# zsyOAOA/ResShift

Measured on AMD Instinct MI355X. Metric: images/sec (1x3x64x64 LR -> 3x256x256, 15-step ResShift sampling loop incl. VQ encode/decode), higher is better.
Workload: dtype f16x2 encoder + UNet (hi+lo fp16 pairs, 3 MFMAs per product: fp32-class) + f16 decoder (parity policy); 1 GPU; realsr_swinunet_realesrgan256: batch 32/GPU x 1 GPU, 1x3x64x64 LR -> 3x256x256, 15 steps, random-init weights; precision_policy=parity, parallelism=dp1 (batch sharded, one RCCL weight broadcast, no data-path collective)

## Files before the change

### include/resshift_hip.h

```cpp
#ifndef RESSHIFT_HIP_H
#define RESSHIFT_HIP_H
#include <stddef.h>
#include <stdint.h>

#ifdef __cplusplus
extern "C" {
#endif

#define RS_PREC_F16 0
#define RS_PREC_F32 1
#define RS_PREC_SPLIT 2
#define RS_MAX_LEVELS 8
#define RS_MAX_STEPS 64
#define RS_MAX_ROWS 64

typedef struct rs_engine rs_engine;

typedef struct rs_unet_config {
    int image_size, in_channels, model_channels, out_channels;
    int n_levels;
    int channel_mult[RS_MAX_LEVELS];
    int num_res_blocks[RS_MAX_LEVELS];
    int n_attn_res;
    int attention_resolutions[RS_MAX_LEVELS];
// ... 46 lines not shown
    float* x;
    float* pred_xstart;
    const float* y;
    const float* mask;
    const float* noise;
    const int* t;
    int B;
    int prec;
    void* stream;
} rs_step_args;

rs_engine* rs_create(const rs_config* cfg);
void rs_destroy(rs_engine* e);
const char* rs_last_error(void);

int rs_load_tensor(rs_engine* e, const char* state_dict_key, const float* host, const int64_t* shape, int ndim);
size_t rs_weight_bytes(rs_engine* e);
int rs_bind_weight_blob(rs_engine* e, void* dev, size_t bytes);
int rs_pack_weights(rs_engine* e);
int rs_bcast_weights(rs_engine* e, void* rccl_comm, int root, void* stream);
int rs_weights_ready(rs_engine* e);

int rs_unet_forward(rs_engine* e, const float* x, const int* t_host, const float* lq, const float* mask, float* out,
                    int B, int H, int W, int Hl, int Wl, int prec, void* stream);
int rs_vq_encode(rs_engine* e, const float* img, float* z, int B, int H, int W, int prec, void* stream);
int rs_vq_decode(rs_engine* e, const float* z, float* img, int32_t* idx_out, int B, int h, int w, int force_not_quantize,
                 int prec, void* stream);
int rs_bicubic(rs_engine* e, const float* y, float* out, int B, int C, int H, int W, int sf, void* stream);
int rs_sample(rs_engine* e, const rs_sample_args* a);
int rs_sample_begin(rs_engine* e, const rs_sample_args* a, float* x_T);
int rs_sample_step(rs_engine* e, const rs_step_args* s);
int rs_sample_end(rs_engine* e, const rs_sample_args* a, const float* x_0);
int rs_film_prewarm(rs_engine* e, const int* timesteps, int n, void* stream);
int rs_axpbypcz(const float* x, const float* z, const float* n, float* y, float a, float b, float c, long long count, void* stream);
int rs_axpbypcz_rows(const float* x, const float* z, const float* n, float* y, const float* a, const float* b, const float* c,
                     long long per_image_count, int B, void* stream);

typedef struct rs_noise_key {
    uint64_t seed;
    uint32_t stream;
    uint32_t reserved;
} rs_noise_key;
int rs_noise_fill(const rs_noise_key* keys, const int* draw, float* out, long long per_image_count, int B, void* stream);
int rs_sample_seeded(rs_engine* e, const rs_sample_args* a, const rs_noise_key* keys);
int rs_sample_begin_seeded(rs_engine* e, const rs_sample_args* a, float* x_T, const rs_noise_key* keys);
int rs_sample_step_seeded(rs_engine* e, const rs_step_args* s, const rs_noise_key* keys);

int rs_tile_accumulate(float* acc, float* count, const float* tile, int B, int C, int H, int W, int h0, int w0, int th, int tw,
                       void* stream);
int rs_tile_finalize(float* acc, const float* count, int B, int C, int H, int W, void* stream);
int rs_window_copy(const float* in, float* out, long long planes, int H, int W, int h0, int w0, int Ho, int Wo, float scale, void* stream);

typedef struct rs_tile_desc {
    const float* src;
    float* acc;
    float* count;
    int H, W, h0, w0, th, tw;
} rs_tile_desc;
int rs_tile_gather(const rs_tile_desc* desc, int n, int C_src, float* out_lq, float* out_mask, int Hp, int Wp, void* stream);
int rs_tile_scatter(const rs_tile_desc* desc, int n, int C, int sf, const float* tiles, int Hp_out, int Wp_out, void* stream);

int rs_tile_accumulate_weighted(float* acc, float* count, const float* tile, int B, int C, int H, int W, int h0, int w0, int th, int tw,
                                int Rh, int Rw, void* stream);
int rs_tile_scatter_weighted(const rs_tile_desc* desc, int n, int C, int sf, const float* tiles, int Hp_out, int Wp_out, int Rh, int Rw,
                             void* stream);

#define RS_COLOR_FIX_WAVELET 1
#define RS_COLOR_FIX_ADAIN 2
size_t rs_color_fix_work_bytes(int B, int C, int H, int W, int sf, int mode);
int rs_color_fix(const float* sr, const float* lq, float* out, int B, int C, int H, int W, int sf, int mode, void* work, size_t work_bytes,
                 void* stream);

int rs_u8_to_input(const void* src_u8_nhwc, float* dst_f32_nchw, int B, int H, int W, int C, void* stream);
int rs_output_to_u8(const float* sr_f32_nchw, const float* lq_f32_nchw, const float* mask_f32_n1hw, void* dst_u8_nhwc, int B, int H,
                    int W, int C, int bgr, void* stream);

size_t rs_arena_bytes(rs_engine* e);
long long rs_last_launch_count(rs_engine* e);
int rs_profile_enable(rs_engine* e, int on);
int rs_profile_get(rs_engine* e, double* out9);
int rs_profile_families(rs_engine* e, double* out, int cap);
int rs_profile_shapes(rs_engine* e, char* buf, int cap);
int rs_debug_enable(rs_engine* e, int on);
int rs_debug_count(rs_engine* e);
int rs_debug_info(rs_engine* e, int i, char* name, int name_cap, int* dims_bchw);
int rs_debug_fetch(rs_engine* e, int i, float* out_nchw_dev, void* stream);
int rs_debug_fetch_rows(rs_engine* e, int i, int b0, int nb, float* out_nchw_dev, void* stream);

int rs_op_conv2d(const void* x0, const void* x1, const float* w_ref_host, const float* bias_host, const void* res, void* y,
                 int B, int Hs, int Ws, int C0, int C1, int Cout, int KH, int KW, int stride, int pad_t, int pad_l, int Ho,
                 int Wo, int up, int act, int in_prec, int out_prec, int force_direct, void* stream);
int rs_op_conv2d_bench(const void* x0, const void* w_packed_dev, const float* bias_dev, const void* res, void* y, int B, int Hs,
                       int Ws, int Cin, int Cout, int KH, int KW, int stride, int pad, int Ho, int Wo, int up, int act, int in_prec,
                       int out_prec, int reps, float* ms_out, void* stream);
int rs_op_conv3x3_halo(const void* x, const float* coef_dev, int act_in, const float* w_ref_host, const float* bias_host, const void* res,
                       void* y, int B, int H, int W, int Cin, int Cout, int prec, float* ystats_dev, void* stream);
int rs_op_conv3x3_wino(const void* x, const float* coef_dev, int act_in, const float* w_ref_host, const float* bias_host, const void* res,
                       void* y, int B, int H, int W, int Cin, int Cout, float* ystats_dev, int reps, float* ms_out, void* stream);
int rs_op_conv3x3_halo_stats_px(int B, int H, int W, int Cin, int Cout, int prec);
int rs_op_gemm_nt(const void* a, const void* b, const float* bias_dev, void* y, int nz, int M, int N, int K, float scale,
                  int in_prec, int out_prec, void* stream);
int rs_op_groupnorm(const void* x, void* y, const float* gamma_host, const float* beta_host, const float* film_dev, int B, int HW,
                    int C, int groups, float eps, int act, int prec, void* stream);
int rs_op_window_attention(const void* qkv, void* out, const float* bias_table_host , int B, int H, int W,
                           int heads, int shift, int prec, void* stream);
int rs_op_window_attention_qkv(const void* x, const void* wqkv_dev, const float* bqkv_dev, const void* wproj_dev, const float* bproj_dev,
                               const void* res, void* out, const float* table_host, int B, int H, int W, int heads, int shift, void* stream);
int rs_op_window_attention_qkv_split(const void* x, const void* wqkv_dev, const float* bqkv_dev, const void* wproj_dev, const float* bproj_dev,
                                     const void* res, void* out, const float* table_host, const float* xcoef_dev, int B, int H, int W, int heads,
                                     int shift, void* stream);
int rs_op_ae_flash_attention(const void* q, const void* k, const void* vt, const float* bv_dev, void* o, int nz, int T, int C, void* stream);
int rs_op_ae_flash_attention_split(const void* q, const void* k, const void* vt, const float* bv_dev, void* o, int nz, int T, int C, void* stream);
int rs_op_swin_mlp(const void* x, const void* w1_dev, const float* b1_dev, const void* w2_dev, const float* b2_dev, const void* res, void* y,
                   int M, int E, int HD, void* stream);
int rs_op_swin_mlp_split(const void* x, const void* w1_dev, const float* b1_dev, const void* w2_dev, const float* b2_dev, const void* res, void* y,
                         int M, int E, int HD, void* stream);
int rs_op_swin_mlp_split_unembed(const void* x, const float* xcoef_dev, const void* w1_dev, const float* b1_dev, const void* w2cat_dev, const float* bcat_dev,
                                 void* y, int M, int HW, int E, int HD, int NO, void* stream);
int rs_op_softmax_rows(const float* s, void* out, long long nrows, int ncols, int out_prec, void* stream);
int rs_op_vq(const float* z, const float* codebook_dev, float* zq, int32_t* idx, long long N, int NE, int D, void* stream);
int rs_op_nchw_to_nhwc(const float* in, void* out, int B, int C, int HW, int out_prec, void* stream);
int rs_op_nhwc_to_nchw(const void* in, float* out, int B, int C, int HW, int in_prec, void* stream);
int rs_op_convert(const void* src, int src_prec, void* dst, int dst_prec, int C, long long npix, void* stream);

#ifdef __cplusplus
}
#endif
#endif
```

### resshift_amd/_lib.py

```python
from __future__ import annotations

import ctypes as C
import os

import torch

HERE = os.path.dirname(os.path.abspath(__file__))
LIB_PATH = os.environ.get("RESSHIFT_HIP_LIB") or os.path.join(HERE, "libresshift_hip.so")

RS_PREC_F16 = 0
RS_PREC_F32 = 1
RS_PREC_SPLIT = 2
RS_MAX_LEVELS = 8
RS_MAX_STEPS = 64
RS_MAX_ROWS = 64
RS_COLOR_FIX_WAVELET = 1
RS_COLOR_FIX_ADAIN = 2
COLOR_FIX_MODES = {"wavelet": RS_COLOR_FIX_WAVELET, "adain": RS_COLOR_FIX_ADAIN}


class UNetConfig(C.Structure):
    _fields_ = [
        ("image_size", C.c_int), ("in_channels", C.c_int), ("model_channels", C.c_int), ("out_channels", C.c_int),
        ("n_levels", C.c_int),
# ... 31 lines not shown
        ("B", C.c_int), ("h", C.c_int), ("w", C.c_int), ("sf", C.c_int), ("steps", C.c_int),
        ("inv_std", C.c_float * RS_MAX_STEPS), ("coef1", C.c_float * RS_MAX_STEPS), ("coef2", C.c_float * RS_MAX_STEPS),
        ("sigma", C.c_float * RS_MAX_STEPS), ("tmap", C.c_int * RS_MAX_STEPS),
        ("prior_scale", C.c_float), ("scale_factor", C.c_float),
        ("prec_encode", C.c_int), ("prec_decode", C.c_int), ("prec_unet", C.c_int * RS_MAX_STEPS),
        ("stream", C.c_void_p),
    ]


class StepArgs(C.Structure):
    _fields_ = [
        ("sched", C.POINTER(SampleArgs)), ("x", C.c_void_p), ("pred_xstart", C.c_void_p), ("y", C.c_void_p), ("mask", C.c_void_p),
        ("noise", C.c_void_p), ("t", C.POINTER(C.c_int)), ("B", C.c_int), ("prec", C.c_int), ("stream", C.c_void_p),
    ]


class TileDesc(C.Structure):
    _fields_ = [("src", C.c_void_p), ("acc", C.c_void_p), ("count", C.c_void_p),
                ("H", C.c_int), ("W", C.c_int), ("h0", C.c_int), ("w0", C.c_int), ("th", C.c_int), ("tw", C.c_int)]


class NoiseKey(C.Structure):
    _fields_ = [("seed", C.c_uint64), ("stream", C.c_uint32), ("reserved", C.c_uint32)]


def noise_keys(keys):
    arr = (NoiseKey * max(1, len(keys)))()
    for d, k in zip(arr, keys):
        if isinstance(k, NoiseKey):
            d.seed, d.stream, d.reserved = k.seed, k.stream, k.reserved
            continue
        seed, stream = (k if isinstance(k, (tuple, list)) else (k, 0))
        if not 0 <= int(stream) < 2 ** 32:
            raise ValueError(f"noise key stream {stream} does not fit 32 bits")
        d.seed, d.stream, d.reserved = int(seed) % 2 ** 64, int(stream), 0
    return arr


_P, _I, _F, _LL, _SZ = C.c_void_p, C.c_int, C.c_float, C.c_longlong, C.c_size_t

SIGNATURES = {
    "rs_create": (_P, [C.POINTER(Config)]),
    "rs_destroy": (None, [_P]),
    "rs_last_error": (C.c_char_p, []),
    "rs_load_tensor": (_I, [_P, C.c_char_p, _P, C.POINTER(C.c_int64), _I]),
    "rs_weight_bytes": (_SZ, [_P]),
    "rs_bind_weight_blob": (_I, [_P, _P, _SZ]),
    "rs_pack_weights": (_I, [_P]),
    "rs_bcast_weights": (_I, [_P, _P, _I, _P]),
    "rs_weights_ready": (_I, [_P]),
    "rs_unet_forward": (_I, [_P, _P, C.POINTER(C.c_int), _P, _P, _P, _I, _I, _I, _I, _I, _I, _P]),
    "rs_vq_encode": (_I, [_P, _P, _P, _I, _I, _I, _I, _P]),
    "rs_vq_decode": (_I, [_P, _P, _P, _P, _I, _I, _I, _I, _I, _P]),
    "rs_bicubic": (_I, [_P, _P, _P, _I, _I, _I, _I, _I, _P]),
    "rs_sample": (_I, [_P, C.POINTER(SampleArgs)]),
    "rs_sample_begin": (_I, [_P, C.POINTER(SampleArgs), _P]),
    "rs_sample_step": (_I, [_P, C.POINTER(StepArgs)]),
    "rs_sample_end": (_I, [_P, C.POINTER(SampleArgs), _P]),
    "rs_film_prewarm": (_I, [_P, C.POINTER(C.c_int), _I, _P]),
    "rs_axpbypcz": (_I, [_P, _P, _P, _P, _F, _F, _F, _LL, _P]),
    "rs_axpbypcz_rows": (_I, [_P, _P, _P, _P, C.POINTER(C.c_float), C.POINTER(C.c_float), C.POINTER(C.c_float), _LL, _I, _P]),
    "rs_noise_fill": (_I, [C.POINTER(NoiseKey), C.POINTER(C.c_int), _P, _LL, _I, _P]),
    "rs_sample_seeded": (_I, [_P, C.POINTER(SampleArgs), C.POINTER(NoiseKey)]),
    "rs_sample_begin_seeded": (_I, [_P, C.POINTER(SampleArgs), _P, C.POINTER(NoiseKey)]),
    "rs_sample_step_seeded": (_I, [_P, C.POINTER(StepArgs), C.POINTER(NoiseKey)]),
    "rs_tile_accumulate": (_I, [_P, _P, _P] + [_I] * 8 + [_P]),
    "rs_tile_finalize": (_I, [_P, _P, _I, _I, _I, _I, _P]),
    "rs_window_copy": (_I, [_P, _P, _LL, _I, _I, _I, _I, _I, _I, _F, _P]),
    "rs_tile_gather": (_I, [C.POINTER(TileDesc), _I, _I, _P, _P, _I, _I, _P]),
    "rs_tile_scatter": (_I, [C.POINTER(TileDesc), _I, _I, _I, _P, _I, _I, _P]),
    "rs_tile_accumulate_weighted": (_I, [_P, _P, _P] + [_I] * 10 + [_P]),
    "rs_tile_scatter_weighted": (_I, [C.POINTER(TileDesc), _I, _I, _I, _P, _I, _I, _I, _I, _P]),
    "rs_color_fix_work_bytes": (_SZ, [_I] * 6),
    "rs_color_fix": (_I, [_P, _P, _P] + [_I] * 6 + [_P, _SZ, _P]),
    "rs_u8_to_input": (_I, [_P, _P, _I, _I, _I, _I, _P]),
    "rs_output_to_u8": (_I, [_P, _P, _P, _P, _I, _I, _I, _I, _I, _P]),
    "rs_arena_bytes": (_SZ, [_P]),
    "rs_last_launch_count": (_LL, [_P]),
    "rs_profile_enable": (_I, [_P, _I]),
    "rs_profile_get": (_I, [_P, C.POINTER(C.c_double)]),
    "rs_profile_families": (_I, [_P, C.POINTER(C.c_double), _I]),
    "rs_profile_shapes": (_I, [_P, C.c_char_p, _I]),
    "rs_debug_enable": (_I, [_P, _I]),
    "rs_debug_count": (_I, [_P]),
    "rs_debug_info": (_I, [_P, _I, C.c_char_p, _I, C.POINTER(C.c_int)]),
    "rs_debug_fetch": (_I, [_P, _I, _P, _P]),
    "rs_debug_fetch_rows": (_I, [_P, _I, _I, _I, _P, _P]),
    "rs_op_conv2d": (_I, [_P, _P, _P, _P, _P, _P] + [_I] * 18 + [_P]),
    "rs_op_conv2d_bench": (_I, [_P, _P, _P, _P, _P] + [_I] * 16 + [C.POINTER(C.c_float), _P]),
    "rs_op_conv3x3_halo_stats_px": (_I, [_I, _I, _I, _I, _I, _I]),
    "rs_op_conv3x3_halo": (_I, [_P, _P, _I, _P, _P, _P, _P, _I, _I, _I, _I, _I, _I, _P, _P]),
    "rs_op_conv3x3_wino": (_I, [_P, _P, _I, _P, _P, _P, _P, _I, _I, _I, _I, _I, _P, _I, C.POINTER(C.c_float), _P]),
    "rs_op_gemm_nt": (_I, [_P, _P, _P, _P, _I, _I, _I, _I, _F, _I, _I, _P]),
    "rs_op_groupnorm": (_I, [_P, _P, _P, _P, _P, _I, _I, _I, _I, _F, _I, _I, _P]),
    "rs_op_window_attention": (_I, [_P, _P, _P, _I, _I, _I, _I, _I, _I, _P]),
    "rs_op_window_attention_qkv": (_I, [_P, _P, _P, _P, _P, _P, _P, _P, _I, _I, _I, _I, _I, _P]),
    "rs_op_window_attention_qkv_split": (_I, [_P, _P, _P, _P, _P, _P, _P, _P, _P, _I, _I, _I, _I, _I, _P]),
    "rs_op_swin_mlp": (_I, [_P, _P, _P, _P, _P, _P, _P, _I, _I, _I, _P]),
    "rs_op_ae_flash_attention": (_I, [_P, _P, _P, _P, _P, _I, _I, _I, _P]),
    "rs_op_ae_flash_attention_split": (_I, [_P, _P, _P, _P, _P, _I, _I, _I, _P]),
    "rs_op_swin_mlp_split": (_I, [_P, _P, _P, _P, _P, _P, _P, _I, _I, _I, _P]),
    "rs_op_swin_mlp_split_unembed": (_I, [_P, _P, _P, _P, _P, _P, _P, _I, _I, _I, _I, _I, _P]),
    "rs_op_softmax_rows": (_I, [_P, _P, _LL, _I, _I, _P]),
    "rs_op_vq": (_I, [_P, _P, _P, _P, _LL, _I, _I, _P]),
    "rs_op_nchw_to_nhwc": (_I, [_P, _P, _I, _I, _I, _I, _P]),
    "rs_op_nhwc_to_nchw": (_I, [_P, _P, _I, _I, _I, _I, _P]),
    "rs_op_convert": (_I, [_P, _I, _P, _I, _I, _LL, _P]),
}

_lib = None


def load() -> C.CDLL:
    global _lib
    if _lib is not None:
        return _lib
    if not os.path.exists(LIB_PATH):
        raise RuntimeError(
            f"{LIB_PATH} is missing: build it with `python -m resshift_amd.build` (hipcc, gfx950). "
            "There is no CPU fallback for the ResShift hot path."
        )
    try:
        lib = C.CDLL(LIB_PATH, mode=C.RTLD_GLOBAL)
    except OSError as e:
        raise RuntimeError(f"cannot load {LIB_PATH}: {e}") from e
    for name, (res, args) in SIGNATURES.items():
        fn = getattr(lib, name)
        fn.restype = res
        fn.argtypes = args
    _lib = lib
    return lib


def last_error() -> str:
    return load().rs_last_error().decode()


def check(rc: int, what: str = "") -> None:
    if rc != 0:
        raise RuntimeError(f"resshift_hip {what} failed (rc={rc}): {last_error()}")


def current_stream_ptr() -> int:
    if torch.cuda.is_available():
        return int(torch.cuda.current_stream().cuda_stream)
    return 0


def window_copy(x, h0=0, w0=0, ho=None, wo=None, scale=1.0, out=None):
    import torch

    if not x.is_cuda:
        raise RuntimeError("window_copy needs a device tensor: the host mirror does not fall back to CPU arithmetic")
    x = x.to(torch.float32).contiguous()
    H, W = x.shape[-2:]
    ho = H if ho is None else ho
    wo = W if wo is None else wo
    planes = x.numel() // (H * W)
    want = (*x.shape[:-2], ho, wo)
    if out is None:
        out = torch.empty(*want, device=x.device, dtype=torch.float32)
    elif out.dtype != torch.float32 or tuple(out.shape) != want or not out.is_contiguous() or out.device != x.device:
        raise ValueError(f"window_copy: `out` must be a contiguous float32 tensor of shape {want} on {x.device} "
                         f"(got {out.dtype}, {tuple(out.shape)}, contiguous={out.is_contiguous()}, {out.device})")
    check(load().rs_window_copy(x.data_ptr(), out.data_ptr(), planes, H, W, h0, w0, ho, wo, float(scale), current_stream_ptr()), "rs_window_copy")
    return out


def _tile_descs(rows):
    arr = (TileDesc * len(rows))()
    for d, r in zip(arr, rows):
        d.src, d.acc, d.count, d.H, d.W, d.h0, d.w0, d.th, d.tw = r
    return arr


# ... 66 lines not shown
```

### resshift_amd/build.py

```python
from __future__ import annotations

import concurrent.futures as cf
import hashlib
import os
import subprocess
import sys

HERE = os.path.dirname(os.path.abspath(__file__))
CSRC = os.path.join(HERE, "csrc")
OBJ = os.path.join(CSRC, "build" + ("_" + hashlib.sha256(os.environ["RS_BUILD_DEFS"].encode()).hexdigest()[:8] if os.environ.get("RS_BUILD_DEFS") else ""))
LIB = os.environ.get("RS_BUILD_OUT") or os.path.join(HERE, "libresshift_hip.so")
SOURCES = ["igemm.hip", "igemm2.hip", "igemm3.hip", "igemm4.hip", "igemm4s.hip", "wino.hip", "igemm_split.hip", "swin_mlp.hip", "direct_conv.hip", "norm_attn.hip", "win_attn_split.hip", "ae_attn.hip", "ae_attn_split.hip", "elementwise.hip", "colorfix.hip", "engine.hip"]
HEADERS = ["common.h", "igemm_common.h", "igemm4_kernel.h", "gn_tail.h", "philox.h", os.path.join("..", "..", "include", "resshift_hip.h")]
HIPCC = os.environ.get("HIPCC", "/opt/rocm/bin/hipcc")
FLAGS = ["--offload-arch=gfx950", "-O3", "-std=c++17", "-fPIC", "-Wno-unused-result"]
FLAGS += [f"-D{d}" for d in os.environ.get("RS_BUILD_DEFS", "").split() if d]
if os.environ.get("RS_BUILD_ABLATE"):
    FLAGS.append("-DRS_SPLIT_ABLATE")


def _digest() -> str:
    h = hashlib.sha256()
    for f in SOURCES + HEADERS:
        with open(os.path.join(CSRC, f), "rb") as fh:
            h.update(fh.read())
    h.update(" ".join(FLAGS).encode())
    return h.hexdigest()


def _compile(src: str) -> str:
    obj = os.path.join(OBJ, src.replace(".hip", ".o"))
    cmd = [HIPCC, *FLAGS, "-c", os.path.join(CSRC, src), "-o", obj]
    r = subprocess.run(cmd, capture_output=True, text=True)
    if r.returncode != 0:
        raise RuntimeError(f"hipcc failed for {src}:\n{r.stderr[-4000:]}")
    return obj


def build(force: bool = False, verbose: bool = True) -> str:
    os.makedirs(OBJ, exist_ok=True)
    stamp = LIB + ".stamp"
    dig = _digest()
    if not force and os.path.exists(LIB) and os.path.exists(stamp) and open(stamp).read().strip() == dig:
        return LIB
    if verbose:
        print(f"[resshift_amd.build] compiling {len(SOURCES)} HIP sources for gfx950 ...", flush=True)
    with cf.ThreadPoolExecutor(max_workers=min(8, len(SOURCES))) as ex:
        objs = list(ex.map(_compile, SOURCES))
    cmd = [HIPCC, "--offload-arch=gfx950", "-shared", "-fPIC", "-o", LIB, *objs]
    r = subprocess.run(cmd, capture_output=True, text=True)
    if r.returncode != 0:
        raise RuntimeError(f"link failed:\n{r.stderr[-4000:]}")
    chk = subprocess.run([sys.executable, "-c", f"import ctypes; ctypes.CDLL({LIB!r})"], capture_output=True, text=True)
    if chk.returncode != 0:
        raise RuntimeError(f"built library does not load:\n{chk.stderr[-2000:]}")
    with open(stamp, "w") as fh:
        fh.write(dig)
    if verbose:
        print(f"[resshift_amd.build] built {LIB}", flush=True)
    return LIB


def build_testhooks(verbose: bool = False) -> str:
    build(force=False, verbose=verbose)
    out = os.path.join(HERE, "libresshift_hip_testhooks.so")
    stamp = out + ".stamp"
    dig = _digest() + "+hooks"
    if os.path.exists(out) and os.path.exists(stamp) and open(stamp).read().strip() == dig:
        return out
    objs = [os.path.join(OBJ, s.replace(".hip", ".o")) for s in SOURCES if s != "engine.hip"]
    if not all(os.path.exists(o) for o in objs):
        os.makedirs(OBJ, exist_ok=True)
        with cf.ThreadPoolExecutor(max_workers=min(8, len(SOURCES))) as ex:
            list(ex.map(_compile, [s for s in SOURCES if s != "engine.hip"]))
    hobj = os.path.join(OBJ, "engine_testhooks.o")
    r = subprocess.run([HIPCC, *FLAGS, "-DRS_TEST_HOOKS", "-c", os.path.join(CSRC, "engine.hip"), "-o", hobj], capture_output=True, text=True)
    if r.returncode != 0:
        raise RuntimeError(f"hipcc failed for engine.hip (-DRS_TEST_HOOKS):\n{r.stderr[-4000:]}")
    r = subprocess.run([HIPCC, "--offload-arch=gfx950", "-shared", "-fPIC", "-o", out, *objs, hobj], capture_output=True, text=True)
    if r.returncode != 0:
        raise RuntimeError(f"link failed:\n{r.stderr[-4000:]}")
    with open(stamp, "w") as fh:
        fh.write(dig)
    return out


if __name__ == "__main__":
    build(force="--force" in sys.argv)
```

### resshift_amd/csrc/common.h

```cpp
#pragma once
#include <hip/hip_runtime.h>
#include <stdint.h>
#include <type_traits>

typedef _Float16 f16;
typedef f16 f16x4 __attribute__((ext_vector_type(4)));
typedef f16 f16x8 __attribute__((ext_vector_type(8)));
typedef float f32x4 __attribute__((ext_vector_type(4)));

enum RsDType { RS_F16 = 0, RS_F32 = 1, RS_F16S = 2 };
enum RsAct { RS_ACT_NONE = 0, RS_ACT_GELU = 1, RS_ACT_SILU = 2 };

static inline size_t rs_dtype_size(int dt) { return dt == RS_F16 ? 2 : 4; }
static inline size_t rs_dtype_chan_bytes(int dt) { return dt == RS_F32 ? 4 : 2; }

struct h2s { unsigned short bits; };
#define RS_LO_SCALE 2048.0f
#define RS_LO_INV 4.8828125e-4f
__host__ __device__ inline void rs_split(float x, f16& hi, f16& lo) {
    hi = (f16)x;
    lo = (f16)((x - (float)hi) * RS_LO_SCALE);
}
__device__ __forceinline__ float rs_join(f16 hi, f16 lo) { return fmaf((float)lo, RS_LO_INV, (float)hi); }
template <typename T> struct Store { static constexpr int PM = 1; static constexpr bool FAST = false; };
// ... 82 lines not shown
    const rs_f32x2 es = {copysignf(e.x, x.x), copysignf(e.y, x.y)};
    return __builtin_elementwise_fma(es, hx, hx);
}
__device__ __forceinline__ void rs_split2(rs_f32x2 v, rs_f16x2& h, rs_f16x2& l) {
    h = __builtin_convertvector(v, rs_f16x2);
    l = __builtin_convertvector((v - __builtin_convertvector(h, rs_f32x2)) * RS_LO_SCALE, rs_f16x2);
}
template <int ACT, bool FAST> __device__ __forceinline__ float rs_act_t(float x) {
    if constexpr (ACT == RS_ACT_GELU) return FAST ? rs_gelu_fast(x) : rs_gelu(x);
    else if constexpr (ACT == RS_ACT_SILU) return FAST ? rs_silu_fast(x) : rs_silu(x);
    else return x;
}

template <typename T> struct Vec8;
template <> struct Vec8<f16> {
    f16x8 v;
    __device__ __forceinline__ void load(const f16* p, int lo = 0) { v = *(const f16x8*)p; }
    __device__ __forceinline__ void store(f16* p, int lo = 0) const { *(f16x8*)p = v; }
    __device__ __forceinline__ float get(int i) const { return (float)v[i]; }
    __device__ __forceinline__ void set(int i, float x) { v[i] = (f16)x; }
};
template <> struct Vec8<float> {
    f32x4 a, b;
    __device__ __forceinline__ void load(const float* p, int lo = 0) { a = *(const f32x4*)p; b = *(const f32x4*)(p + 4); }
    __device__ __forceinline__ void store(float* p, int lo = 0) const { *(f32x4*)p = a; *(f32x4*)(p + 4) = b; }
    __device__ __forceinline__ float get(int i) const { return i < 4 ? a[i] : b[i - 4]; }
    __device__ __forceinline__ void set(int i, float x) { if (i < 4) a[i] = x; else b[i - 4] = x; }
};
template <> struct Vec8<h2s> {
    f16x8 h, l;
    __device__ __forceinline__ void load(const h2s* p, int lo) { h = *(const f16x8*)p; l = *(const f16x8*)((const f16*)p + lo); }
    __device__ __forceinline__ void store(h2s* p, int lo) const { *(f16x8*)p = h; *(f16x8*)((f16*)p + lo) = l; }
    __device__ __forceinline__ float get(int i) const { return rs_join(h[i], l[i]); }
    __device__ __forceinline__ void set(int i, float x) { f16 a, b; rs_split(x, a, b); h[i] = a; l[i] = b; }
};


struct GNTail {
    const float* gamma; const float* beta;
    const float* film;
    int film_ld;
    float* coef;
    unsigned* ticket;
    int expected;
    int C, groups, HW;
    float eps;
    const float* st0; int S0, ld0, n0;
    const float* st1; int S1, ld1;
    const float* stg; int Sg;
};


struct IGemmParams {
    const void* x0;
    const void* x1;
    const void* w;
    const float* bias;
    const void* res;
    void* y;
    int C0, C1, ld0, ld1;
    int B, Hs, Ws, up;
    int Ho, Wo, KH, KW, stride, pad_t, pad_l;
    int Cout, ldy, ldres;
    int M, Ktot;
    int act;
    float out_scale;
    long long bs_x0, bs_w, bs_y, bs_res;
    int splitk;
    float* partial;
    unsigned x_bytes, w_bytes;
    int sh_howo, sh_wo;
    int dbg;
    int no_halo;
    const float* xcoef;
    int xact;
    float* ystats;
    int ystats_ld;
    GNTail tail;
    const void* sx; const void* sw; const float* sbias;
    int sC, sld;
    unsigned sx_bytes, sw_bytes;
    int osc, ooy, oox;
    const void* ww;
};

#if defined(__HIPCC__)
__device__ __forceinline__ long long rs_out_m(const IGemmParams& p, long long m) {
    if (p.osc != 2) return m;
    const int hw = p.Ho * p.Wo;
    const int b = (int)(m / hw), r = (int)(m - (long long)b * hw);
    const int oy = r / p.Wo, ox = r - oy * p.Wo;
    return ((long long)b * (2 * p.Ho) + 2 * oy + p.ooy) * (2 * p.Wo) + 2 * ox + p.oox;
}
#endif

struct DirectConvParams {
    const void* x0; const void* x1;
    const float* w;
    const float* bias;
    void* y;
    int C0, C1, ld0, ld1;
    int B, Hs, Ws, up, Ho, Wo, KH, KW, stride, pad_t, pad_l;
    int Cout, ldy, act;
};

struct GNParams {
    const void* x; void* y;
    const float* gamma; const float* beta;
    const float* film;
    int film_ld;
    float* partial;
    int B, HW, C, ldx, ldy, S, groups;
    float eps; int act;
    float* coef;
    const float* cpartial;
    int cp_ld;
    const float* cpartial2;
    int cp2_ld, cp2_S, cp_n0;
    unsigned* ticket;
};

struct WinAttnParams {
    const void* qkv;
    void* out;
    const float* bias_t;
    const float* bias_n;
    const float* bias_c;
    int B, H, W, heads, shift, ldq, ldo;
    float scale;
    const void* x;
    const void* wqkv;
    const float* bqkv;
    int ldx;
    const void* wproj;
    const float* bproj;
    const void* res;
    int ldres;
    const float* xcoef;
    float* ystats;
    int ystats_ld;
    GNTail tail;
};
```

### resshift_amd/csrc/engine.hip

```cpp
#include "common.h"
#include "../../include/resshift_hip.h"
#include <dlfcn.h>
#include <algorithm>
#include <array>
#include <cmath>
#include <cstdio>
#include <cstring>
#include <functional>
#include <map>
#include <string>
#include <unordered_map>
#include <vector>

extern "C" {
int rs_igemm_launch(const IGemmParams* p, int in_dt, int out_dt, int nz, hipStream_t st);
int rs_igemm_splitk_plan(int M, int Cout, int Ktot, int in_dt);
int rs_igemm4_pick(const IGemmParams* p, int in_dt, int out_dt, int nz, int* TW, int* BC);
int rs_igemm4_plan(const IGemmParams* p, int in_dt, int out_dt, int nz, int* TW, int* BC, int* SEG, int* SK);
int rs_igemm4_stats_px(const IGemmParams* p, int in_dt);
int rs_wino_plan(const IGemmParams* p, int in_dt, int out_dt, int nz);
int rs_wino_launch(const IGemmParams* p, hipStream_t st);
size_t rs_wino_weight_bytes(int Cin, int Cout);
float rs_wino_pack(const float* w_ref, int Cin, int Cout, void* dst);
int rs_wino_stats_px();
int rs_wino_tiles(const IGemmParams* p);
int rs_igemm_split_stats_px(const IGemmParams* p, int splitk);
int rs_direct_conv_launch(const DirectConvParams* p, int in_dt, int out_dt, hipStream_t st);
int rs_head_conv_launch(const void* x, int in_dt, const float* coef_dev, const float* w_dev, const float* bias_dev, float* y, int B, int H, int W, int C,
                        int ldx, int Cout, int ldy, hipStream_t st);
int rs_groupnorm_launch(const GNParams* p, int dt, int apply_slabs, hipStream_t st);
int rs_win_attn_launch(const WinAttnParams* p, int dt, hipStream_t st);
int rs_softmax_rows_launch(const float* s, void* out, int out_dt, long long nrows, int ncols, long long lds_, long long ldo, hipStream_t st);
int rs_nchw_to_nhwc_launch(const float* in, void* out, int out_dt, int B, int C, int HW, int ldo, int coff, float scale, hipStream_t st);
int rs_nhwc_to_nchw_launch(const void* in, int in_dt, float* out, int B, int C, int HW, int ldi, int coff, hipStream_t st);
int rs_axpbypcz_launch(const float* x, const float* z, const float* n, float* y, float a, float b, float c, long long cnt, hipStream_t st);
int rs_axpbypcz_rows_launch(const float* x, const float* z, const float* n, float* y, const float* a, const float* b, const float* c, long long per,
                            int B, hipStream_t st);
int rs_axpbypcz_seeded_launch(const float* x, const float* z, float* y, const float* a, const float* b, const float* c, const rs_noise_key* keys,
                              const rs_noise_key* keys_dev, const int* draw, long long per, int B, hipStream_t st);
int rs_film_gather_launch(const float* const* rows, int B, int total, float* out, hipStream_t st);
int rs_nchw_to_nhwc_rows_launch(const float* in, void* out, int out_dt, int B, int C, int HW, int ldo, int coff, const float* scale, hipStream_t st);
int rs_clamp_launch(float* x, float lo, float hi, long long cnt, hipStream_t st);
int rs_win_attn_qkv_supported(int heads, int E);
int rs_win_attn_qkv_launch(const WinAttnParams* p, hipStream_t st);
int rs_win_attn_qkv_split_launch(const WinAttnParams* p, hipStream_t st);
int rs_ae_flash_supported(int C, int T);
int rs_ae_flash_launch(const void* q, int ldq, const void* k, int ldk, const void* vt, const float* bv, void* o, int ldo, int nz, int T, int C,
                       float scale, hipStream_t st);
int rs_ae_flash_split_supported(int C, int T);
int rs_ae_flash_split_launch(const void* q, int ldq, const void* k, int ldk, const void* vt, const float* bv, void* o, int ldo, int nz, int T, int C,
                             float scale, hipStream_t st);
int rs_swin_mlp_supported(int E, int HD);
int rs_swin_mlp_split_launch(const void* x, const void* w1, const float* b1, const void* w2, const float* b2, const void* res, void* y, int M, int ldx,
                             int ldres, int ldy, int E, int HD, const float* xcoef, int HW, float* ystats, int ystats_ld, const GNTail* tail, hipStream_t st);
int rs_swin_mlp_split_launch_n(const void* x, const void* w1, const float* b1, const void* w2, const float* b2, const void* res, void* y, int M, int ldx,
                               int ldres, int ldy, int E, int HD, int NO, const float* xcoef, int HW, float* ystats, int ystats_ld, const GNTail* tail,
                               hipStream_t st);
int rs_swin_mlp_split_unembed_supported(int E, int HD, int NO);
int rs_swin_mlp_launch(const void* x, const void* w1, const float* b1, const void* w2, const float* b2, const void* res, void* y, int M, int ldx,
                       int ldres, int ldy, int E, int HD, const float* xcoef, int HW, float* ystats, int ystats_ld, hipStream_t st);
int rs_small_linear_launch(const float* x, const float* w, const float* bias, float* y, int R, int K, int N, int silu_in, int silu_out, hipStream_t st);
int rs_bicubic_launch(const float* in, void* out, int out_dt, int B, int C, int H, int W, int sf, int ldo, hipStream_t st);
int rs_vq_launch(const float* z, const float* codebook, float* zq, int* idx, long long N, int NE, int D, hipStream_t st);
int rs_copy_channels_launch(const void* src, int lds_, void* dst, int ldd, int C, long long npix, int dt, hipStream_t st);
int rs_convert_launch(const void* src, int src_dt, void* dst, int dst_dt, int C, long long npix, hipStream_t st);
}

namespace {

thread_local std::string g_err;
int fail(const std::string& m) { g_err = m; return -1; }

struct HostTensor { std::vector<float> data; std::vector<int64_t> shape; };

template <class FH, class FL>
static void frag_major_fill(int N, int K, f16* dst, bool with_lo, FH hi, FL lo) {
    const int KS = K / 32, parts = with_lo ? 2 : 1;
    for (int nb = 0; nb < N / 16; ++nb)
        for (int ks = 0; ks < KS; ++ks)
            for (int lane = 0; lane < 64; ++lane)
                for (int e = 0; e < 8; ++e) {
                    const int n = 16 * nb + (lane & 15), k = 32 * ks + 8 * (lane >> 4) + e;
                    const size_t o = (((size_t)(nb * KS + ks) * parts) * 64 + lane) * 8 + e;
                    dst[o] = hi(n, k);
                    if (with_lo) dst[o + 512] = lo(n, k);
                }
}
static void rs_pack_frag_major(const float* w, int N, int K, f16* out16, f16* outsplit) {
    if (out16) frag_major_fill(N, K, out16, false, [&](int n, int k) { return (f16)w[(size_t)n * K + k]; }, [&](int, int) { return (f16)0.f; });
    if (outsplit)
        frag_major_fill(N, K, outsplit, true, [&](int n, int k) { f16 h, l; rs_split(w[(size_t)n * K + k], h, l); return h; },
                        [&](int n, int k) { f16 h, l; rs_split(w[(size_t)n * K + k], h, l); return l; });
}
static void* frag_major_from_device_rows(const void* wdev, int N, int K, int ld, int lo_off) {
    std::vector<f16> rows((size_t)N * ld), out((size_t)N * K * (lo_off >= 0 ? 2 : 1));
    if (hipMemcpy(rows.data(), wdev, rows.size() * sizeof(f16), hipMemcpyDeviceToHost) != hipSuccess) return nullptr;
    frag_major_fill(N, K, out.data(), lo_off >= 0, [&](int n, int k) { return rows[(size_t)n * ld + k]; },
                    [&](int n, int k) { return rows[(size_t)n * ld + (lo_off >= 0 ? lo_off : 0) + k]; });
    void* d = nullptr;
    if (hipMalloc(&d, out.size() * sizeof(f16)) != hipSuccess) return nullptr;
    (void)hipMemcpy(d, out.data(), out.size() * sizeof(f16), hipMemcpyHostToDevice);
    return d;
}

struct View {
    void* p = nullptr; int B = 0, H = 0, W = 0, C = 0, ld = 0, dt = RS_F16;
    float* st = nullptr; int stS = 0, stld = 0;
    int st_prod = -1;
    float* st2 = nullptr; int st2S = 0, st2ld = 0, st_n0 = 0;
// ... 215 lines not shown
            (void)hipEventRecord(e0, st);
        }
        if (sp) check(rs_win_attn_qkv_split_launch(&p, st), "win_attn_qkv_split");
        else check(rs_win_attn_qkv_launch(&p, st), "win_attn_qkv");
        if (e1) (void)hipEventRecord(e1, st);
    }
    void ae_flash(const void* q, int ldq, const void* k, int ldk, const void* vt, const float* bv, void* o, int ldo, int nz, int T, int C, float scale,
                  int dt = RS_F16) {
        const int sp = dt == RS_F16S;
        const double fl = 4.0 * (double)nz * (double)T * (double)T * (double)C;
        igemm_flops[sp ? 2 : 0] += fl;
        fam_note(sp ? F_AEFLASH_S : F_AEFLASH, fl, T, T, C, nz);
        igemm_bytes += (sp ? 4.0 : 2.0) * 4.0 * (double)nz * T * C;
        ++igemm_launches;
        hipEvent_t e0, e1;
        bracket(prof, st, e0, e1);
        if (sp) check(rs_ae_flash_split_launch(q, ldq, k, ldk, vt, bv, o, ldo, nz, T, C, scale, st), "ae_flash_attn_split");
        else check(rs_ae_flash_launch(q, ldq, k, ldk, vt, bv, o, ldo, nz, T, C, scale, st), "ae_flash_attn");
        if (e1) (void)hipEventRecord(e1, st);
    }
    void swin_mlp(const void* x, const void* w1, const float* b1, const void* w2, const float* b2, const void* res, void* y, int M, int ldx,
                  int ldres, int ldy, int E, int HD, const float* xcoef = nullptr, int HW = 0, int dt = RS_F16, float* ystats = nullptr,
                  int ystats_ld = 0, const GNTail* tail = nullptr, int NO = 0) {
        const int sp = dt == RS_F16S;
        if (NO <= 0) NO = E;
        const double fl = 2.0 * (double)M * ((double)E * HD + (double)NO * (NO != E ? HD + E : HD));
        igemm_flops[sp ? 2 : 0] += fl;
        fam_note(sp ? F_SWINMLP_S : F_SWINMLP, fl, M, NO, HD);
        igemm_bytes += (sp ? 4.0 : 2.0) * ((double)M * (E * ((res || NO != E) ? 2.0 : 1.0) + NO) + (double)E * HD + (double)NO * (NO != E ? HD + E : HD));
        ++igemm_launches;
        hipEvent_t e0 = nullptr, e1 = nullptr;
        if (prof && prof->on) {
            if (prof->used + 2 > prof->ev.size()) {
                const size_t old = prof->ev.size();
                prof->ev.resize(old + 1024);
                for (size_t i = old; i < prof->ev.size(); ++i) (void)hipEventCreate(&prof->ev[i]);
            }
            e0 = prof->ev[prof->used++]; e1 = prof->ev[prof->used++];
            (void)hipEventRecord(e0, st);
        }
        if (sp) check(rs_swin_mlp_split_launch_n(x, w1, b1, w2, b2, res, y, M, ldx, ldres, ldy, E, HD, NO, xcoef, HW, ystats, ystats_ld, tail, st), "swin_mlp_split");
        else check(rs_swin_mlp_launch(x, w1, b1, w2, b2, res, y, M, ldx, ldres, ldy, E, HD, xcoef, HW, ystats, ystats_ld, st), "swin_mlp");
        if (e1) (void)hipEventRecord(e1, st);
    }
};

}

#ifdef RS_TEST_HOOKS
static bool rs_fake_device() {
    static const bool fake = []() {
        if (!getenv("RS_FAKE_DEVICE")) return false;
        int n = 0;
        const hipError_t e = hipGetDeviceCount(&n);
        return e == hipErrorNoDevice || (e == hipSuccess && n == 0);
    }();
    return fake;
}
#else
static constexpr bool rs_fake_device() { return false; }
#endif

struct rs_engine {
    rs_config cfg;
    std::unordered_map<std::string, HostTensor> host;
    Blob blob;
    size_t blob_bytes = 0;
    bool bound = false, ready = false;
    std::string build_err;
    std::string split_err;
    bool split_ok = true;
    std::vector<unsigned char> big_w;
    int conv_count = 0;
    unsigned char* big_w_dev = nullptr;
    bool big(const ConvW& c) const { return c.idx >= 0 && c.idx < (int)big_w.size() && big_w[c.idx] != 0; }
    Arena arena;
    long long last_launches = 0;
    Exec::Prof prof, prof_gn;
    double last_flops[3] = {0.0, 0.0, 0.0}, last_igemm_ms = 0.0, last_igemm_bytes = 0.0, last_gn_ms = 0.0, last_gn_bytes = 0.0;
    double last_fam[Exec::F_COUNT][3] = {};
    std::string last_shapes;
    long long last_igemm_launches = 0, last_gn_launches = 0;
    bool debug = false;
    std::vector<TraceRec> trace;
    rs_noise_key* keys_dev = nullptr; size_t keys_cap = 0;
    const rs_noise_key* stage_keys(const rs_noise_key* keys, int B, hipStream_t st) {
        if (rs_fake_device()) return (const rs_noise_key*)(uintptr_t)4096;
        if ((size_t)B > keys_cap) {
            (void)hipStreamSynchronize(st);
            if (keys_dev) (void)hipFree(keys_dev);
            keys_dev = nullptr; keys_cap = 0;
            if (hipMalloc((void**)&keys_dev, (size_t)B * sizeof(rs_noise_key)) != hipSuccess) return nullptr;
            keys_cap = (size_t)B;
        }
        if (hipMemcpyWithStream(keys_dev, keys, (size_t)B * sizeof(rs_noise_key), hipMemcpyHostToDevice, st) != hipSuccess) return nullptr;
        return keys_dev;
    }
    char* cap_base = nullptr; size_t cap_bytes = 0; bool cap_host = false;
    void free_capture() {
        if (cap_base) { if (cap_host) free(cap_base); else (void)hipFree(cap_base); }
        cap_base = nullptr; cap_bytes = 0; trace.clear();
    }
    std::vector<TailPlan> tail_plan;
    std::vector<UBlock> in_blocks, out_blocks;
    ResBlockW mid_res1, mid_res2; BasicLayerW mid_swin;
    std::vector<ConvW> fe_convs, fe_downs;
    GNW out_norm; ConvW out_conv;
    ConvW te0, te2;
    std::vector<int> skip_ch, h_ch;
    int film_total = 0, fe_out_ch = 0;
    std::vector<ResBlockW*> film_blocks;
    std::map<int, float*> film_cache;
    ConvW enc_in, enc_out, dec_in, dec_out, quant_conv, post_quant_conv;
    std::vector<AELevel> enc_levels, dec_levels;
    ResBlockW enc_mid1, enc_mid2, dec_mid1, dec_mid2;
    AttnW enc_attn, dec_attn;
    GNW enc_norm, dec_norm;
    float* codebook = nullptr;

    std::map<std::string, std::function<bool(HostTensor&)>> derived;
    const HostTensor* find(const std::string& k) {
        auto it = host.find(k);
        if (it == host.end()) {
            auto d = derived.find(k);
            if (d != derived.end()) {
                HostTensor t;
                if (d->second(t)) it = host.emplace(k, std::move(t)).first;
            }
        }
        if (it == host.end()) { if (build_err.empty()) build_err = "missing state_dict key: " + k; return nullptr; }
        return &it->second;
    }
    float* add_f32(const std::string& key, size_t n) {
        return (float*)blob.add(n * sizeof(float), [&](char* dst) {
            const HostTensor* t = find(key);
            if (!t) return;
            if (t->data.size() != n) { if (build_err.empty()) build_err = "bad size for " + key; return; }
            memcpy(dst, t->data.data(), n * sizeof(float));
        });
    }
    ConvW add_conv(const std::string& prefix, int Cin, int Cout, int KH, int KW, bool has_bias = true, bool force_direct = false, bool head = false) {
        ConvW c; c.Cin = Cin; c.Cout = Cout; c.KH = KH; c.KW = KW;
        c.idx = conv_count++;
        if ((int)big_w.size() < conv_count) big_w.resize(conv_count, 0);
        const int cidx = c.idx;
        c.direct = force_direct;
        c.CinP = c.direct ? Cin : (Cin + 7) / 8 * 8;
        const int CinP = c.CinP;
        const size_t K = (size_t)KH * KW * CinP, n = (size_t)KH * KW * Cin * Cout, np = K * Cout;
        const std::string wkey = prefix + ".weight";
        auto get = [&]() -> const float* {
            const HostTensor* t = find(wkey);
            if (!t) return nullptr;
            if (t->data.size() != n) { if (build_err.empty()) build_err = "bad size for " + wkey; return nullptr; }
            return t->data.data();
        };
        if (c.direct) {
            c.wd = (float*)blob.add(n * 4, [&](char* dst) {
                const float* w = get(); if (!w) return;
                float* o = (float*)dst;
                for (int co = 0; co < Cout; ++co)
                    for (int ci = 0; ci < Cin; ++ci)
                        for (int t = 0; t < KH * KW; ++t)
                            o[((size_t)t * Cin + ci) * Cout + co] = w[((size_t)co * Cin + ci) * KH * KW + t];
            });
        } else {
// ... 345 lines not shown
    ResBlockW add_resnet(const std::string& p, int Cin, int Cout) {
        ResBlockW r; r.Cin = Cin; r.Cout = Cout;
        r.n1 = add_gn(p + ".norm1", Cin);
        r.c1 = add_conv(p + ".conv1", Cin, Cout, 3, 3);
        r.n2 = add_gn(p + ".norm2", Cout);
        r.c2 = add_conv(p + ".conv2", Cout, Cout, 3, 3);
        r.has_skip = Cin != Cout;
        if (r.has_skip) r.skip = add_conv(p + ".nin_shortcut", Cin, Cout, 1, 1);
        return r;
    }
    AttnW add_attn(const std::string& p, int C) {
        AttnW a; a.C = C;
        a.norm = add_gn(p + ".norm", C);
        a.q = add_conv(p + ".q", C, C, 1, 1);
        a.k = add_conv(p + ".k", C, C, 1, 1);
        a.v = add_conv(p + ".v", C, C, 1, 1);
        a.proj = add_conv(p + ".proj_out", C, C, 1, 1);
        return a;
    }
    void build_ae() {
        const rs_ae_config& a = cfg.ae;
        enc_levels.clear(); dec_levels.clear();
        enc_in = add_conv("encoder.conv_in", a.in_channels, a.ch, 3, 3);
        int block_in = a.ch;
        for (int l = 0; l < a.n_levels; ++l) {
            AELevel L;
            block_in = a.ch * (l == 0 ? 1 : a.ch_mult[l - 1]);
            const int block_out = a.ch * a.ch_mult[l];
            for (int i = 0; i < a.num_res_blocks[l]; ++i) {
                L.blocks.push_back(add_resnet("encoder.down." + std::to_string(l) + ".block." + std::to_string(i), block_in, block_out));
                block_in = block_out;
            }
            if (l != a.n_levels - 1) {
                L.has_resample = true;
                L.resample = add_conv("encoder.down." + std::to_string(l) + ".downsample.conv", block_in, block_in, 3, 3);
            }
            enc_levels.push_back(L);
        }
        enc_mid1 = add_resnet("encoder.mid.block_1", block_in, block_in);
        enc_attn = add_attn("encoder.mid.attn_1", block_in);
        enc_mid2 = add_resnet("encoder.mid.block_2", block_in, block_in);
        enc_norm = add_gn("encoder.norm_out", block_in);
        enc_out = add_conv("encoder.conv_out", block_in, a.z_channels, 3, 3, true, false, true);
        quant_conv = add_conv("quant_conv", a.z_channels, a.embed_dim, 1, 1, true, true);
        post_quant_conv = add_conv("post_quant_conv", a.embed_dim, a.z_channels, 1, 1, true, true);
        block_in = a.ch * a.ch_mult[a.n_levels - 1];
        dec_in = add_conv("decoder.conv_in", a.z_channels, block_in, 3, 3);
        dec_mid1 = add_resnet("decoder.mid.block_1", block_in, block_in);
        dec_attn = add_attn("decoder.mid.attn_1", block_in);
        dec_mid2 = add_resnet("decoder.mid.block_2", block_in, block_in);
        dec_levels.resize(a.n_levels);
        for (int l = a.n_levels - 1; l >= 0; --l) {
            AELevel L;
            const int block_out = a.ch * a.ch_mult[l];
            for (int i = 0; i <= a.num_res_blocks[l]; ++i) {
                L.blocks.push_back(add_resnet("decoder.up." + std::to_string(l) + ".block." + std::to_string(i), block_in, block_out));
                block_in = block_out;
            }
            if (l != 0) {
                L.has_resample = true;
                L.resample = add_conv("decoder.up." + std::to_string(l) + ".upsample.conv", block_in, block_in, 3, 3);
                L.has_upf = add_upfold("decoder.up." + std::to_string(l) + ".upsample.conv", block_in, L.upf);
            }
            dec_levels[l] = L;
        }
        dec_norm = add_gn("decoder.norm_out", block_in);
        dec_out = add_conv("decoder.conv_out", block_in, a.out_ch, 3, 3, true, false, true);
        codebook = add_f32("quantize.embedding.weight", (size_t)a.n_embed * a.embed_dim);
    }
    size_t build(char* base, bool fill) {
        blob.base = base; blob.off = 0; blob.fill = fill;
        build_err.clear();
        split_err.clear();
        if (fill) blob.staging.assign(blob_bytes, 0);
        (void)blob.add(256, [](char*) {});
        conv_count = 0;
        if (fill) std::fill(big_w.begin(), big_w.end(), 0);
        if (cfg.has_unet) build_unet();
        if (cfg.has_ae) build_ae();
        big_w_dev = (unsigned char*)blob.add((size_t)conv_count, [&](char* dst) { memcpy(dst, big_w.data(), (size_t)conv_count); });
        return (blob.off + 255) & ~(size_t)255;
    }

    static IGemmParams conv_params(const ConvW& w, const View& x, const View* x1, const View& y, int stride, int pad_t, int pad_l, int up,
                                   int act, const View* res, float out_scale) {
        const int C1 = x1 ? x1->C : 0;
        IGemmParams p{};
        p.x0 = x.p; p.x1 = x1 ? x1->p : nullptr; p.w = w.w_for(x.dt); p.bias = w.bias;
        p.res = res ? res->p : nullptr; p.y = y.p;
        p.C0 = x.C; p.C1 = C1; p.ld0 = x.ld; p.ld1 = x1 ? x1->ld : 0;
        p.B = x.B; p.Hs = x.H; p.Ws = x.W; p.up = up; p.Ho = y.H; p.Wo = y.W; p.KH = w.KH; p.KW = w.KW;
        p.stride = stride; p.pad_t = pad_t; p.pad_l = pad_l; p.Cout = w.Cout; p.ldy = y.ld; p.ldres = res ? res->ld : 0;
        p.M = y.B * y.H * y.W; p.Ktot = w.KH * w.KW * (x.C + C1); p.act = act; p.out_scale = out_scale;
        p.splitk = 1;
        p.ww = (x.dt == RS_F16S && !x1) ? w.ww : nullptr;
        return p;
    }
    bool halo_conv(const ConvW& w, const View& x, const View& y, const View* res, int* sk = nullptr, int* seg = nullptr, bool folded = false,
                   bool* wino = nullptr) const {
        if (wino) *wino = false;
        if (w.direct || (x.dt != RS_F16 && x.dt != RS_F16S) || y.dt != x.dt || x.C != w.CinP) return false;
        if (x.dt == RS_F16S && big(w)) return false;
        const IGemmParams p = conv_params(w, x, nullptr, y, 1, 1, 1, 1, 0, res, 1.f);
        if (!folded && rs_wino_plan(&p, x.dt, y.dt, 1)) {
            if (sk) *sk = 1;
            if (seg) *seg = 0;
            if (wino) *wino = true;
            return true;
        }
        int tw, bc, sg = 0, k = 1;
        if (!rs_igemm4_plan(&p, x.dt, y.dt, 1, &tw, &bc, &sg, &k)) return false;
        if (sk) *sk = k;
        if (seg) *seg = sg;
        return true;
    }
    void conv(Exec& ex, const ConvW& w, const View& x, const View* x1, const View& y, int stride, int pad_t, int pad_l, int up,
              int act, const View* res, float out_scale = 1.f, const float* xcoef = nullptr, int xact = RS_ACT_NONE,
              const ConvW* skw = nullptr, const View* skx = nullptr) {
        const int C1 = x1 ? x1->C : 0;
        int splitk = 1;
        float* partial = nullptr;
        if (!w.direct) {
            const int M = y.B * y.H * y.W;
            int sk4 = 1;
            if (!x1 && w.KH == 3 && stride == 1 && pad_t == 1 && pad_l == 1 && up == 1 && halo_conv(w, x, y, res, &sk4, nullptr, skw != nullptr)) splitk = sk4;
            else splitk = rs_igemm_splitk_plan(M, w.Cout, w.KH * w.KW * (x.C + C1), x.dt);
            if (splitk > 1) partial = (float*)ex.raw((size_t)splitk * M * w.Cout * sizeof(float));
        }
        View xcat;
        if (!w.direct && x1 && x.dt == RS_F16S) {
            xcat = ex.T(x.B, x.H, x.W, x.C + C1, x.dt);
            if (!ex.dry) {
                ex.check(rs_copy_channels_launch(x.p, x.ld, xcat.p, xcat.ld, x.C, x.pixels(), x.dt, ex.st), "concat copy");
                ex.check(rs_copy_channels_launch(x1->p, x1->ld, xcat.slice(x.C, C1).p, xcat.ld, C1, x.pixels(), x.dt, ex.st), "concat copy");
            }
            conv(ex, w, xcat, nullptr, y, stride, pad_t, pad_l, up, act, res, out_scale);
            return;
        }
        if (ex.dry) return;
        if (x.C + C1 != w.CinP) { if (!ex.err) { ex.err = -3; g_err = "conv input channels do not match the packed weights"; } return; }
        if (w.direct) {
            DirectConvParams p{};
            p.x0 = x.p; p.x1 = x1 ? x1->p : nullptr; p.w = w.wd; p.bias = w.bias; p.y = y.p;
            p.C0 = x.C; p.C1 = C1; p.ld0 = x.ld; p.ld1 = x1 ? x1->ld : 0;
            p.B = x.B; p.Hs = x.H; p.Ws = x.W; p.up = up; p.Ho = y.H; p.Wo = y.W; p.KH = w.KH; p.KW = w.KW;
            p.stride = stride; p.pad_t = pad_t; p.pad_l = pad_l; p.Cout = w.Cout; p.ldy = y.ld; p.act = act;
            if (res) { ex.err = -3; g_err = "direct conv has no residual path"; return; }
            ex.check(rs_direct_conv_launch(&p, x.dt, y.dt, ex.st), "direct_conv");
        } else {
            IGemmParams p = conv_params(w, x, x1, y, stride, pad_t, pad_l, up, act, res, out_scale);
            p.no_halo = (x.dt == RS_F16S && big(w)) ? 1 : 0;
            p.splitk = splitk; p.partial = partial;
            p.xcoef = xcoef; p.xact = xact;
            if (skw) { p.sx = skx->p; p.sw = skw->w_for(x.dt); p.sbias = skw->bias; p.sC = skx->C; p.sld = skx->ld; p.ww = nullptr; }
            if (y.st) {
                const bool halo = !x1 && w.KH == 3 && stride == 1 && pad_t == 1 && pad_l == 1 && up == 1 && halo_conv(w, x, y, res, nullptr, nullptr, skw != nullptr);
                if (halo || (!x1 && x.dt == RS_F16S && y.dt == RS_F16S)) { p.ystats = y.st; p.ystats_ld = y.stld; }
                else { ex.err = -3; g_err = "output statistics requested from a conv whose kernel cannot produce them"; return; }
                (void)ex.fill_tail(y.st_prod, y.B, p.tail);
            }
            if (!p.w) { ex.err = -3; g_err = "weights for this precision were not packed (enable_f16/enable_f32/enable_split)"; return; }
            ex.igemm(p, x.dt, y.dt, 1, "igemm");
        }
    }
    void zero(Exec& ex, const View& v) {
        if (ex.dry) return;
        const hipError_t e = hipMemsetAsync(v.p, 0, (size_t)v.B * v.H * v.W * v.ld * rs_dtype_size(v.dt), ex.st);
        ex.check(e == hipSuccess ? 0 : -1, "memset");
    }
    void conv3(Exec& ex, const ConvW& w, const View& x, const View& y, const View* res = nullptr, int act = 0, const float* xcoef = nullptr,
               int xact = RS_ACT_NONE, const ConvW* skw = nullptr, const View* skx = nullptr) {
        conv(ex, w, x, nullptr, y, 1, 1, 1, 1, act, res, 1.f, xcoef, xact, skw, skx);
    }
    bool skip_fold(const Exec& ex, const ResBlockW& r, const View& X, const View& h1, const View& Y) const {
        static const bool on = []() { const char* e = getenv("RS_SKIP_FOLD"); return !(e && e[0] == '0'); }();
        static const bool fold = []() { const char* e = getenv("RS_GN_CONV_FOLD"); return !(e && e[0] == '0'); }();
        static const bool on16 = []() { const char* e = getenv("RS_SKIP_FOLD_F16"); return !(e && e[0] == '0'); }();
        if (!on || !fold || !r.has_skip || (X.dt != RS_F16S && !(X.dt == RS_F16 && on16)) || Y.dt != X.dt) return false;
// ... 908 lines not shown

int rs_bcast_weights(rs_engine* e, void* rccl_comm, int root, void* stream) {
    if (!e || !e->bound || !rccl_comm) return fail("rs_bcast_weights: bind a weight blob first and pass an RCCL communicator");
    typedef int (*bcast_t)(const void*, void*, size_t, int, int, void*, hipStream_t);
    static bcast_t fn = []() -> bcast_t {
        void* h = dlopen("librccl.so", RTLD_NOW | RTLD_GLOBAL);
        if (!h) h = dlopen("librccl.so.1", RTLD_NOW | RTLD_GLOBAL);
        return h ? (bcast_t)dlsym(h, "ncclBroadcast") : nullptr;
    }();
    if (!fn) return fail("rs_bcast_weights: librccl.so (ncclBroadcast) not found");
    const int rc = fn(e->blob.base, e->blob.base, e->blob_bytes,  1, root, rccl_comm, (hipStream_t)stream);
    if (rc != 0) return fail("rs_bcast_weights: ncclBroadcast failed (ncclResult_t " + std::to_string(rc) + ")");
    e->ready = false;
    return 0;
}

int rs_pack_weights(rs_engine* e) {
    if (!e || !e->bound) return fail("rs_pack_weights: bind a weight blob first");
    char* base = e->blob.base;
    e->build(base, true);
    e->collect_film_blocks();
    if (!e->build_err.empty()) { e->blob.staging.clear(); e->blob.staging.shrink_to_fit(); return fail(e->build_err); }
    e->split_ok = e->split_err.empty();
    {
        const uint32_t flags = e->split_ok ? 1u : 0u;
        memcpy(e->blob.staging.data(), &flags, sizeof flags);
    }
    if (hipMemcpy(base, e->blob.staging.data(), e->blob_bytes, hipMemcpyHostToDevice) != hipSuccess) return fail("hipMemcpy of weight blob failed");
    e->blob.staging.clear(); e->blob.staging.shrink_to_fit();
    e->blob.fill = false;
    e->host.clear();
    for (auto& kv : e->film_cache) (void)hipFree(kv.second);
    e->film_cache.clear();
    e->ready = true;
    return 0;
}

int rs_weights_ready(rs_engine* e) {
    if (!e || !e->bound) return fail("rs_weights_ready: bind a weight blob first");
    uint32_t flags = 0;
    if (rs_fake_device()) { e->split_ok = true; e->ready = true; return 0; }
    if (hipMemcpy(&flags, e->blob.base, sizeof flags, hipMemcpyDeviceToHost) != hipSuccess) return fail("rs_weights_ready: cannot read the blob header");
    e->split_ok = (flags & 1u) != 0;
    if (e->conv_count > 0 && e->big_w_dev &&
        hipMemcpy(e->big_w.data(), e->big_w_dev, (size_t)e->conv_count, hipMemcpyDeviceToHost) != hipSuccess) return fail("rs_weights_ready: cannot read the per-layer flags");
    for (auto& kv : e->film_cache) (void)hipFree(kv.second);
    e->film_cache.clear();
    e->ready = true;
    return 0;
}

size_t rs_arena_bytes(rs_engine* e) { return e ? e->arena.cap : 0; }

int rs_profile_enable(rs_engine* e, int on) { if (!e) return -1; e->prof.on = on != 0; return 0; }
int rs_profile_get(rs_engine* e, double* out) {
    if (!e || !out) return -1;
    out[0] = e->last_flops[0]; out[1] = e->last_flops[1]; out[2] = e->last_igemm_ms; out[3] = (double)e->last_igemm_launches;
    out[4] = e->last_igemm_bytes; out[5] = e->last_flops[2];
    out[6] = e->last_gn_ms; out[7] = (double)e->last_gn_launches; out[8] = e->last_gn_bytes;
    return 0;
}

int rs_profile_families(rs_engine* e, double* out, int cap) {
    if (!e || !out || cap < 3 * Exec::F_COUNT) return -1;
    for (int f = 0; f < Exec::F_COUNT; ++f) { out[3 * f] = e->last_fam[f][0]; out[3 * f + 1] = e->last_fam[f][1]; out[3 * f + 2] = e->last_fam[f][2]; }
    return Exec::F_COUNT;
}

int rs_profile_shapes(rs_engine* e, char* buf, int cap) {
    if (!e) return -1;
    const int need = (int)e->last_shapes.size() + 1;
    if (buf && cap > 0) { const int n = std::min(cap - 1, need - 1); memcpy(buf, e->last_shapes.data(), n); buf[n] = 0; }
    return need;
}

int rs_debug_enable(rs_engine* e, int on) {
    if (!e) return -1;
    e->debug = on != 0;
    if (!e->debug) {
        if (e->cap_base && !e->cap_host) (void)hipDeviceSynchronize();
        e->free_capture();
    }
    e->trace.clear();
    return 0;
}
int rs_debug_count(rs_engine* e) { return e ? (int)e->trace.size() : 0; }
int rs_debug_info(rs_engine* e, int i, char* name, int cap, int* dims ) {
    if (!e || i < 0 || i >= (int)e->trace.size()) return -1;
    const TraceRec& t = e->trace[i];
    snprintf(name, cap, "%s", t.name.c_str());
    dims[0] = t.B; dims[1] = t.C; dims[2] = t.H; dims[3] = t.W;
    return 0;
}
int rs_debug_fetch(rs_engine* e, int i, float* out_nchw, void* stream) {
    if (!e || i < 0 || i >= (int)e->trace.size() || !e->cap_base) return -1;
    const TraceRec& t = e->trace[i];
    const size_t bytes = (size_t)t.B * t.C * t.H * t.W * sizeof(float);
    return hipMemcpyAsync(out_nchw, e->cap_base + t.off, bytes, hipMemcpyDefault, (hipStream_t)stream) == hipSuccess ? 0 : -1;
}
int rs_debug_fetch_rows(rs_engine* e, int i, int b0, int nb, float* out_nchw, void* stream) {
    if (!e || i < 0 || i >= (int)e->trace.size() || !e->cap_base) return -1;
    const TraceRec& t = e->trace[i];
    if (b0 < 0 || nb < 1 || b0 > t.B - nb) return -2;
    const size_t per = (size_t)t.C * t.H * t.W * sizeof(float);
    return hipMemcpyAsync(out_nchw, e->cap_base + t.off + (size_t)b0 * per, (size_t)nb * per, hipMemcpyDefault, (hipStream_t)stream) == hipSuccess ? 0 : -1;
}
long long rs_last_launch_count(rs_engine* e) { return e ? e->last_launches : 0; }

int rs_unet_forward(rs_engine* e, const float* x, const int* t_host, const float* lq, const float* mask, float* out, int B, int H, int W,
                    int Hl, int Wl, int prec, void* stream) {
    if (!e || !e->cfg.has_unet) return fail("engine has no UNet");
    {
        const int sh = e->cfg.unet.n_levels - 1;
        if ((H % (8 << sh)) || (W % (8 << sh))) return fail("UNet input H/W must be multiples of 8*2^(levels-1)");
    }
    hipStream_t st = (hipStream_t)stream;
    if (!e->ready) return fail("weights are not ready");
    if (B < 1 || !x || !out || !t_host) return fail("rs_unet_forward: bad batch / null tensor");
    if (e->cfg.unet.cond_lq && !lq) return fail("rs_unet_forward: this UNet is conditioned on lq (cond_lq) but lq is NULL");
    if (e->cfg.unet.cond_mask && !mask) return fail("rs_unet_forward: this UNet is conditioned on a mask (cond_mask) but mask is NULL");
    if (e->cfg.unet.cond_lq && e->fe_convs.empty() && (Hl != H || Wl != W))
        return fail("rs_unet_forward: without a feature extractor lq must have the latent resolution");
    if (!e->fe_convs.empty() && ((Hl >> (int)e->fe_convs.size()) != H || (Wl >> (int)e->fe_convs.size()) != W))
        return fail("rs_unet_forward: lq resolution does not match the feature extractor's down-sampling");
    bool mixed = false;
    for (int b = 1; b < B; ++b) mixed |= t_host[b] != t_host[0];
    if (mixed && B > RS_MAX_ROWS) return fail("rs_unet_forward: unequal timesteps in a batch of more than RS_MAX_ROWS (" + std::to_string(RS_MAX_ROWS) + ") images");
    std::vector<const float*> rows(mixed ? B : 1);
    for (size_t b = 0; b < rows.size(); ++b)
        if (!(rows[b] = e->film_row(t_host[b], st))) return fail("FiLM table allocation failed");
    return e->run(st, [&](Exec& ex) {
        View feat; const View* fp = nullptr;
        if (!e->fe_convs.empty()) { feat = e->feature_extract(ex, lq, mask, B, Hl, Wl, prec); fp = &feat; }
        if (!mixed) e->unet_body(ex, x, 1.0f, fp, lq, mask, Hl, Wl, out, B, H, W, prec, rows[0]);
        else e->unet_body(ex, x, 1.0f, fp, lq, mask, Hl, Wl, out, B, H, W, prec, e->film_table(ex, rows.data(), B), e->film_total);
    });
}

int rs_vq_encode(rs_engine* e, const float* img, float* z, int B, int H, int W, int prec, void* stream) {
    if (!e || !e->cfg.has_ae) return fail("engine has no autoencoder");
    hipStream_t st = (hipStream_t)stream;
    return e->run(st, [&](Exec& ex) {
        View in = ex.T(B, H, W, e->enc_in.CinP, prec);
        e->zero(ex, in);
        if (!ex.dry) ex.check(rs_nchw_to_nhwc_launch(img, in.p, prec, B, e->cfg.ae.in_channels, H * W, in.ld, 0, 1.f, st), "img->nhwc");
        e->encode_body(ex, in, z, prec);
    });
}

int rs_vq_decode(rs_engine* e, const float* z, float* img, int32_t* idx_out, int B, int h, int w, int force_not_quantize, int prec,
                 void* stream) {
    if (!e || !e->cfg.has_ae) return fail("engine has no autoencoder");
    hipStream_t st = (hipStream_t)stream;
    return e->run(st, [&](Exec& ex) { e->decode_body(ex, z, 1.0f, img, idx_out, B, h, w, force_not_quantize, prec); });
}

int rs_bicubic(rs_engine* e, const float* y, float* out, int B, int C, int H, int W, int sf, void* stream) {
    if (!e) return fail("null engine");
    hipStream_t st = (hipStream_t)stream;
    const bool was_ready = e->ready;
    e->ready = true;
    const int rc = e->run(st, [&](Exec& ex) {
        View t = ex.T(B, H * sf, W * sf, C, RS_F32);
        if (ex.dry) return;
        ex.check(rs_bicubic_launch(y, t.p, RS_F32, B, C, H, W, sf, t.ld, st), "bicubic");
        ex.check(rs_nhwc_to_nchw_launch(t.p, RS_F32, out, B, C, H * sf * W * sf, t.ld, 0, st), "bicubic->nchw");
// ... 307 lines not shown
            }
    void* wdev = dev_copy(o.data(), o.size() * 2);
    float* bias = bias_host ? (float*)dev_copy(bias_host, Cout * 4) : nullptr;
    IGemmParams p{};
    p.x0 = x; p.w = wdev; p.bias = bias; p.res = res; p.y = y; p.C0 = Cin; p.ld0 = Cin; p.B = B; p.Hs = H; p.Ws = W; p.up = 1; p.Ho = H; p.Wo = W;
    p.KH = 3; p.KW = 3; p.stride = 1; p.pad_t = 1; p.pad_l = 1; p.Cout = Cout; p.ldy = Cout; p.ldres = Cout; p.M = B * H * W; p.Ktot = (int)K;
    p.out_scale = 1.f; p.splitk = 1; p.xcoef = coef_dev; p.xact = act_in;
    int tw, bc, seg, sk, rc;
    float* part = nullptr;
    if (!rs_igemm4_plan(&p, prec, prec, 1, &tw, &bc, &seg, &sk)) rc = fail("shape is not eligible for the halo kernel");
    else {
        p.splitk = sk;
        if (sk > 1) { (void)hipMalloc((void**)&part, (size_t)sk * p.M * Cout * sizeof(float)); p.partial = part; }
        p.ystats = ystats_dev; p.ystats_ld = Cout;
        rc = rs_igemm_launch(&p, prec, prec, 1, st);
    }
    (void)hipStreamSynchronize(st);
    if (part) (void)hipFree(part);
    if (wdev) (void)hipFree(wdev);
    if (bias) (void)hipFree(bias);
    return rc;
}

int rs_op_conv3x3_wino(const void* x, const float* coef_dev, int act_in, const float* w_ref_host, const float* bias_host, const void* res, void* y,
                       int B, int H, int W, int Cin, int Cout, float* ystats_dev, int reps, float* ms_out, void* stream) {
    hipStream_t st = (hipStream_t)stream;
    if (Cin < 32 || (Cin % 32) || Cout < 32 || (Cout % 32)) return fail("wino kernel: channels in multiples of 32");
    std::vector<char> packed(rs_wino_weight_bytes(Cin, Cout));
    const float mx = rs_wino_pack(w_ref_host, Cin, Cout, packed.data());
    if (!(mx < 30.0f)) return fail("wino kernel: |U| >= 30");
    void* wdev = dev_copy(packed.data(), packed.size());
    float* bias = bias_host ? (float*)dev_copy(bias_host, Cout * 4) : nullptr;
    IGemmParams p{};
    p.x0 = x; p.ww = wdev; p.bias = bias; p.res = res; p.y = y; p.C0 = Cin; p.ld0 = Cin; p.B = B; p.Hs = H; p.Ws = W; p.up = 1; p.Ho = H; p.Wo = W;
    p.KH = 3; p.KW = 3; p.stride = 1; p.pad_t = 1; p.pad_l = 1; p.Cout = Cout; p.ldy = Cout; p.ldres = Cout; p.M = B * H * W; p.Ktot = 9 * Cin;
    p.out_scale = 1.f; p.splitk = 1; p.xcoef = coef_dev; p.xact = act_in; p.ystats = ystats_dev; p.ystats_ld = Cout;
    int rc = 0;
    float* stamps = nullptr;
    const int ntile = rs_wino_tiles(&p);
    p.dbg = 64;
    if (const char* ab = getenv("RS_WINO_ABL")) p.dbg |= atoi(ab);
    if (getenv("RS_WINO_STAMPS")) { (void)hipMalloc((void**)&stamps, (size_t)ntile * 16 * sizeof(float)); (void)hipMemset(stamps, 0, (size_t)ntile * 16 * sizeof(float)); p.partial = stamps; }
    if (!rs_wino_plan(&p, RS_F16S, RS_F16S, 1)) rc = fail("shape is not eligible for the wino kernel");
    else {
        rc = rs_wino_launch(&p, st);
        if (rc) fail("wino launch failed");
        if (stamps) {
            (void)hipStreamSynchronize(st);
            std::vector<float> hs((size_t)ntile * 16);
            (void)hipMemcpy(hs.data(), stamps, hs.size() * sizeof(float), hipMemcpyDeviceToHost);
            double wide[16] = {}; int nw = 0;
            for (int t = 0; t < ntile; ++t) {
                for (int i = 0; i < 16; ++i) wide[i] += hs[(size_t)t * 16 + i];
                ++nw;
            }
            static const char* nm[8] = {"prologue", "wait+barrier", "halo issue", "B operand", "MFMA steps", "conversion", "epilogue", "total"};
            fprintf(stderr, "[wino phases] %dx%dx%d %d->%d, mean cycles of wave 0 over %d workgroups:", B, H, W, Cin, Cout, nw);
            for (int i = 0; i < 8; ++i) fprintf(stderr, " %s %.0f", nm[i], wide[i] / std::max(1, nw));
            static const char* nq[6] = {"drain", "barrier-1", "exchange writes", "barrier-2", "transform + stores", "statistics"};
            fprintf(stderr, "  | epilogue:");
            for (int i = 0; i < 6; ++i) fprintf(stderr, " %s %.0f", nq[i], wide[8 + i] / std::max(1, nw));
            fprintf(stderr, "\n");
        }
        if (!rc && reps > 0) {
            hipEvent_t e0, e1;
            (void)hipEventCreate(&e0); (void)hipEventCreate(&e1);
            (void)hipEventRecord(e0, st);
            for (int i = 0; i < reps; ++i) rc |= rs_wino_launch(&p, st);
            (void)hipEventRecord(e1, st);
            (void)hipEventSynchronize(e1);
            float ms = 0.f;
            (void)hipEventElapsedTime(&ms, e0, e1);
            if (ms_out) *ms_out = ms / (float)reps;
            (void)hipEventDestroy(e0); (void)hipEventDestroy(e1);
        }
    }
    (void)hipStreamSynchronize(st);
    if (stamps) (void)hipFree(stamps);
    if (wdev) (void)hipFree(wdev);
    if (bias) (void)hipFree(bias);
    return rc;
}

int rs_op_conv3x3_halo_stats_px(int B, int H, int W, int Cin, int Cout, int prec) {
    IGemmParams p{};
    p.C0 = Cin; p.ld0 = Cin; p.B = B; p.Hs = H; p.Ws = W; p.up = 1; p.Ho = H; p.Wo = W;
    p.KH = 3; p.KW = 3; p.stride = 1; p.pad_t = 1; p.pad_l = 1; p.Cout = Cout; p.ldy = Cout; p.ldres = Cout; p.M = B * H * W; p.Ktot = 9 * Cin;
    return rs_igemm4_stats_px(&p, prec);
}

int rs_op_gemm_nt(const void* a, const void* b, const float* bias_dev, void* y, int nz, int M, int N, int K, float scale, int in_prec,
                  int out_prec, void* stream) {
    IGemmParams p{};
    p.x0 = a; p.w = b; p.bias = bias_dev; p.y = y; p.C0 = K; p.ld0 = K; p.B = 1; p.Hs = M; p.Ws = 1; p.up = 1; p.Ho = M; p.Wo = 1;
    p.KH = 1; p.KW = 1; p.stride = 1; p.Cout = N; p.ldy = N; p.M = M; p.Ktot = K; p.out_scale = scale;
    p.bs_x0 = (long long)M * K; p.bs_w = (long long)N * K; p.bs_y = (long long)M * N;
    const int rc = rs_igemm_launch(&p, in_prec, out_prec, nz, (hipStream_t)stream);
    if (rc) fail("igemm launch rejected the shape");
    return rc;
}

int rs_op_groupnorm(const void* x, void* y, const float* gamma_host, const float* beta_host, const float* film_dev, int B, int HW, int C,
                    int groups, float eps, int act, int prec, void* stream) {
    hipStream_t st = (hipStream_t)stream;
    float* g = (float*)dev_copy(gamma_host, C * 4);
    float* bt = (float*)dev_copy(beta_host, C * 4);
    int S = std::max(1, std::min(64, 1024 / std::max(1, B)));
    S = std::max(1, std::min(S, HW / 8));
    const int S2 = std::max(1, std::min(HW / 8, std::max(1, 2048 / std::max(1, B))));
    float* partial = nullptr;
    (void)hipMalloc((void**)&partial, (size_t)B * S * groups * 2 * 4);
    GNParams p{};
    p.x = x; p.y = y; p.gamma = g; p.beta = bt; p.film = film_dev; p.partial = partial; p.B = B; p.HW = HW; p.C = C; p.ldx = C; p.ldy = C;
    p.S = S; p.groups = groups; p.eps = eps; p.act = act;
    const int nk = rs_groupnorm_launch(&p, prec, S2, st);
    const int rc = nk < 0 ? nk : 0;
    if (rc) fail("groupnorm launch rejected the shape");
    (void)hipStreamSynchronize(st);
    (void)hipFree(g); (void)hipFree(bt); (void)hipFree(partial);
    return rc;
}

int rs_op_window_attention(const void* qkv, void* out, const float* table_host, int B, int H, int W, int heads, int shift, int prec,
                           void* stream) {
    hipStream_t st = (hipStream_t)stream;
    std::vector<float> bt((size_t)heads * 64 * 64);
    for (int h = 0; h < heads; ++h)
        for (int j = 0; j < 64; ++j)
            for (int i = 0; i < 64; ++i) {
                const int idx = ((i >> 3) - (j >> 3) + 7) * 15 + ((i & 7) - (j & 7) + 7);
                bt[((size_t)h * 64 + j) * 64 + i] = table_host[(size_t)idx * heads + h];
            }
    float* d = (float*)dev_copy(bt.data(), bt.size() * 4);
    std::vector<float> bn(bt.size());
    for (int h = 0; h < heads; ++h)
        for (int i = 0; i < 64; ++i)
            for (int j = 0; j < 64; ++j) bn[((size_t)h * 64 + i) * 64 + j] = bt[((size_t)h * 64 + j) * 64 + i];
    float* dn = (float*)dev_copy(bn.data(), bn.size() * 4);
    WinAttnParams p{};
    p.bias_n = dn;
    p.qkv = qkv; p.out = out; p.bias_t = d; p.B = B; p.H = H; p.W = W; p.heads = heads; p.shift = shift; p.ldq = 3 * heads * 32;
    p.ldo = heads * 32; p.scale = 1.0f / std::sqrt(32.0f);
    const int rc = rs_win_attn_launch(&p, prec, st);
    if (rc) fail("window attention launch rejected the shape");
    (void)hipStreamSynchronize(st);
    (void)hipFree(d);
    (void)hipFree(dn);
    return rc;
}

int rs_op_window_attention_qkv(const void* x, const void* wqkv_dev, const float* bqkv_dev, const void* wproj_dev, const float* bproj_dev,
                               const void* res, void* out, const float* table_host, int B, int H, int W, int heads, int shift, void* stream) {
    hipStream_t st = (hipStream_t)stream;
    std::vector<float> bn((size_t)heads * 64 * 64);
    for (int h = 0; h < heads; ++h)
        for (int i = 0; i < 64; ++i)
            for (int j = 0; j < 64; ++j) {
                const int idx = ((i >> 3) - (j >> 3) + 7) * 15 + ((i & 7) - (j & 7) + 7);
                bn[((size_t)h * 64 + i) * 64 + j] = table_host[(size_t)idx * heads + h];
            }
    float* dn = (float*)dev_copy(bn.data(), bn.size() * 4);
    std::vector<float> bc((size_t)heads * 256, 0.0f);
    for (int h = 0; h < heads; ++h)
        for (int k = 0; k < 225; ++k) bc[(size_t)h * 256 + k] = table_host[(size_t)k * heads + h] * 1.44269504088896f;
    float* dc = (float*)dev_copy(bc.data(), bc.size() * 4);
    WinAttnParams p{};
// ... 92 lines not shown
```

### resshift_amd/csrc/igemm.hip

```cpp
#include "igemm_common.h"
#include <algorithm>

namespace {

using namespace igemm_detail;

template <typename TI, typename TO, int BP, int BC>
__global__ __launch_bounds__(256) void igemm_kernel(IGemmParams p) {
    constexpr int CH = MfmaOps<TI>::CH;
    constexpr int BK = 8 * CH;
    constexpr int XR = BP / 32;
    constexpr int WR = BC / 32;
    constexpr int FP = BP / 32;
    constexpr int FC = BC / 32;
    static_assert(BP % 32 == 0 && BC % 32 == 0, "tile");

    extern __shared__ __attribute__((aligned(16))) char smem[];
    char* xs_base = smem;
    char* ws_base = smem + 2 * BP * 128;

    const int tid = threadIdx.x;
    const int kc = tid & 7;
    const int r0 = tid >> 3;
    const int lane = tid & 63;
// ... 234 lines not shown
        const int n = (int)(q - m * (p.Cout >> 2)) * 4;
        f32x4 s = *(const f32x4*)(p.partial + m * p.Cout + n);
        for (int zz = 1; zz < p.splitk; ++zz) {
            const f32x4 t = *(const f32x4*)(p.partial + zz * slab + m * p.Cout + n);
            s[0] += t[0]; s[1] += t[1]; s[2] += t[2]; s[3] += t[3];
        }
        float v[4];
#pragma unroll
        for (int r = 0; r < 4; ++r) {
            float t = s[r] * p.out_scale;
            if (p.bias) t += p.bias[n + r];
            v[r] = epi_act<TO>(t, p.act);
        }
        if (p.res) {
            const TO* rp = (const TO*)p.res + m * p.ldres * PM + n;
            if ((p.ldres & 3) == 0) {
                float rv[4];
                Out4<TO>::load(rp, rv, p.ldres);
#pragma unroll
                for (int r = 0; r < 4; ++r) v[r] += rv[r];
            } else {
                for (int r = 0; r < 4; ++r) v[r] += rs_ld<TO>(rp + r, p.ldres);
            }
        }
        TO* yp = (TO*)p.y + m * p.ldy * PM + n;
        if ((p.ldy & 3) == 0) Out4<TO>::store(yp, v, p.ldy);
        else for (int r = 0; r < 4; ++r) rs_st<TO>(yp + r, p.ldy, v[r]);
    }
}

void pick_tile(int M, int Cout, int& BP, int& BC) {
    auto waste = [&](int bc) { return ((Cout + bc - 1) / bc) * bc - Cout; };
    int best = 128, bw = waste(128);
    if (waste(160) < bw) { best = 160; bw = waste(160); }
    if (waste(192) < bw) { best = 192; bw = waste(192); }
    if (Cout <= 64) best = 64;
    BC = best;
    BP = (M <= 64 * 48) ? 64 : 128;
}

template <typename TI, typename TO, int BP, int BC>
hipError_t launch_cfg(const IGemmParams& p, int nz, hipStream_t st) {
    const int tiles = ((p.M + BP - 1) / BP) * ((p.Cout + BC - 1) / BC);
    dim3 grid(tiles, 1, p.splitk > 1 ? p.splitk : nz);
    const size_t lds = 2 * (BP + BC) * 128;
    static RsAttrFlags attr_flags;
    if (attr_flags.need()) {
        (void)hipFuncSetAttribute((const void*)igemm_kernel<TI, TO, BP, BC>, hipFuncAttributeMaxDynamicSharedMemorySize, (int)lds);
    }
    hipLaunchKernelGGL((igemm_kernel<TI, TO, BP, BC>), grid, dim3(256), lds, st, p);
    if (p.splitk > 1) {
        const long long nq = (long long)p.M * (p.Cout >> 2);
        const unsigned blocks = (unsigned)std::min<long long>((nq + 255) / 256, 4096);
        hipLaunchKernelGGL((splitk_reduce_kernel<TO>), dim3(blocks), dim3(256), 0, st, p);
    }
    return hipGetLastError();
}

template <typename TI, typename TO>
hipError_t launch_t(const IGemmParams& p, int nz, hipStream_t st) {
    int BP, BC;
    pick_tile(p.M, p.Cout, BP, BC);
    const bool small_m = BP == 64;
    switch (BC) {
        case 64: return small_m ? launch_cfg<TI, TO, 64, 64>(p, nz, st) : launch_cfg<TI, TO, 128, 64>(p, nz, st);
        case 160: return small_m ? launch_cfg<TI, TO, 64, 160>(p, nz, st) : launch_cfg<TI, TO, 128, 160>(p, nz, st);
        case 192: return small_m ? launch_cfg<TI, TO, 64, 192>(p, nz, st) : launch_cfg<TI, TO, 128, 192>(p, nz, st);
        default: return small_m ? launch_cfg<TI, TO, 64, 128>(p, nz, st) : launch_cfg<TI, TO, 128, 128>(p, nz, st);
    }
}

}

extern "C" int rs_igemm2_pick(int M, int Cout, int Kbytes, int nz, int* BP, int* BC);
extern "C" int rs_igemm2_launch(const IGemmParams* pp, int in_dt, int out_dt, int BP, int BC, int nz, hipStream_t st);
extern "C" int rs_igemm3_pick(int M, int Cout, int Ktot, int in_dt, int nz, int splitk, int* BC);
extern "C" int rs_igemm3_launch(const IGemmParams* pp, int out_dt, int BC, hipStream_t st);
extern "C" int rs_igemm4_pick(const IGemmParams* pp, int in_dt, int out_dt, int nz, int* TW, int* BC);
extern "C" int rs_igemm4_launch(const IGemmParams* pp, int in_dt, int TW, int BC, hipStream_t st);
extern "C" int rs_wino_plan(const IGemmParams* pp, int in_dt, int out_dt, int nz);
extern "C" int rs_wino_launch(const IGemmParams* pp, hipStream_t st);
extern "C" void rs_igemm_split_pick(int M, int Cout, int nz, int* BP, int* BC);
extern "C" int rs_igemm_split_launch(const IGemmParams* pp, int out_dt, int nz, hipStream_t st);

extern "C" int rs_splitk_reduce_launch(const IGemmParams* pp, int out_dt, hipStream_t st) {
    const IGemmParams& p = *pp;
    const long long nq = (long long)p.M * (p.Cout >> 2);
    const unsigned blocks = (unsigned)std::min<long long>((nq + 255) / 256, 4096);
    if (out_dt == RS_F16) hipLaunchKernelGGL((splitk_reduce_kernel<f16>), dim3(blocks), dim3(256), 0, st, p);
    else if (out_dt == RS_F16S) hipLaunchKernelGGL((splitk_reduce_kernel<h2s>), dim3(blocks), dim3(256), 0, st, p);
    else hipLaunchKernelGGL((splitk_reduce_kernel<float>), dim3(blocks), dim3(256), 0, st, p);
    return hipGetLastError() == hipSuccess ? 0 : -1;
}

extern "C" int rs_igemm_splitk_plan(int M, int Cout, int Ktot, int in_dt) {
    int BP, BC;
    if (in_dt == RS_F16S) {
        rs_igemm_split_pick(M, Cout, 1, &BP, &BC);
        const int tiles = ((M + BP - 1) / BP) * ((Cout + BC - 1) / BC);
        const int nk = (Ktot + 63) / 64;
        if (tiles >= 200 || nk < 16 || (Cout & 3)) return 1;
        int s = std::min((256 + tiles - 1) / tiles, 16);
        s = std::min(s, nk / 8);
        return std::max(s, 1);
    }
    pick_tile(M, Cout, BP, BC);
    if (Cout > 64) {
        int bp2 = 0, bc2 = 0;
        if (rs_igemm2_pick(M, Cout, Ktot * (in_dt == RS_F16 ? 2 : 4), 1, &bp2, &bc2)) { BP = bp2 == 133 ? 64 : (bp2 == 256 || bp2 == 131) ? 256 : 128; BC = bc2; }
    }
    const int tiles = ((M + BP - 1) / BP) * ((Cout + BC - 1) / BC);
    const int bk = in_dt == RS_F16 ? 64 : 32;
    const int nk = (Ktot + bk - 1) / bk;
    if (tiles >= (BP == 64 ? 400 : 200) || nk < 16 || (Cout & 3)) return 1;
    static const int target = []() { const char* e = getenv("RS_SPLITK_TARGET"); return e ? atoi(e) : 512; }();
    static const int minst = []() { const char* e = getenv("RS_SPLITK_MINSTAGES"); return e ? atoi(e) : 8; }();
    int s = (target + tiles - 1) / tiles;
    s = std::min(s, 16);
    s = std::min(s, nk / minst);
    return std::max(s, 1);
}

extern "C" int rs_igemm_launch(const IGemmParams* pp, int in_dt, int out_dt, int nz, hipStream_t st) {
    IGemmParams p = *pp;
    const int ch = in_dt == RS_F32 ? 4 : 8;
    if ((p.C0 % ch) || (p.C1 % ch) || (p.ld0 % ch) || (p.C1 && (p.ld1 % ch)) || p.M <= 0 || p.Cout <= 0) return -2;
    if (p.up != 1 && p.up != 2) return -2;
    if (p.splitk < 1) p.splitk = 1;
    if (p.splitk > 1 && (nz != 1 || !p.partial || (p.Cout & 3))) return -2;
    if (p.osc != 0 && p.osc != 1 && (p.osc != 2 || p.res || (p.ystats && in_dt != RS_F16S) || p.splitk > 1 || nz != 1 || p.up != 1 || p.stride != 1 || p.C1 != 0)) return -2;
    if (rs_wino_plan(&p, in_dt, out_dt, nz)) return rs_wino_launch(&p, st);
    {
        int tw4 = 0, bc4 = 0;
        if (rs_igemm4_pick(&p, in_dt, out_dt, nz, &tw4, &bc4)) return rs_igemm4_launch(&p, in_dt, tw4, bc4, st);
        if (p.xcoef || p.sx) return -2;
    }
    if (in_dt == RS_F16S) return rs_igemm_split_launch(&p, out_dt, nz, st);
    static const bool use_v2 = []() { const char* e = getenv("RS_IGEMM_V2"); return !(e && e[0] == '0'); }();
    int bp2 = 0, bc2 = 0;
    int bc3 = 0;
    if (use_v2 && p.C1 == 0 && (out_dt == RS_F16 || out_dt == RS_F32) && rs_igemm3_pick(p.M, p.Cout, p.Ktot, in_dt, nz, p.splitk, &bc3)) return rs_igemm3_launch(&p, out_dt, bc3, st);
    if (use_v2 && p.C1 == 0 && rs_igemm2_pick(p.M, p.Cout, p.Ktot * (in_dt == RS_F16 ? 2 : 4), nz * p.splitk, &bp2, &bc2)) return rs_igemm2_launch(&p, in_dt, out_dt, bp2, bc2, nz, st);
    hipError_t e;
    if (in_dt == RS_F16 && out_dt == RS_F16) e = launch_t<f16, f16>(p, nz, st);
    else if (in_dt == RS_F16 && out_dt == RS_F32) e = launch_t<f16, float>(p, nz, st);
    else if (in_dt == RS_F32 && out_dt == RS_F32) e = launch_t<float, float>(p, nz, st);
    else return -2;
    return e == hipSuccess ? 0 : -1;
}
```

### resshift_amd/csrc/igemm_split.hip

```cpp
#include "igemm_common.h"
#include "gn_tail.h"
#include <algorithm>
#include <type_traits>

extern "C" int rs_splitk_reduce_launch(const IGemmParams* p, int out_dt, hipStream_t st);
extern "C" int rs_splitk_reduce_stats_launch(const IGemmParams* p, int out_dt, hipStream_t st);

namespace {

using namespace igemm_detail;

typedef __attribute__((address_space(3))) void* lds_ptr_t;

__device__ __forceinline__ void lds_dma16(__amdgpu_buffer_rsrc_t r, char* lds, unsigned voff) {
    __builtin_amdgcn_raw_ptr_buffer_load_lds(r, (lds_ptr_t)lds, 16, voff, 0, 0, 0);
}

template <int N> __device__ __forceinline__ void wait_vmcnt() { asm volatile("s_waitcnt vmcnt(%0)" ::"n"(N) : "memory"); }

#ifdef RS_SPLIT_ABLATE
__device__ long long g_igs_clk[4 * 8192];
#define RS_IGS_STAMP(k) if (threadIdx.x == 0 && blockIdx.x < 8192 && blockIdx.z == 0) g_igs_clk[4 * blockIdx.x + (k)] = clock64()
#else
#define RS_IGS_STAMP(k)
#endif
template <typename TO, int BP, int BC, int NWV, bool PIPE, int ABL = 0>
__global__ __launch_bounds__(64 * NWV, NWV == 8 ? 2 : 1) void igemm_split_kernel(IGemmParams p) {
    RS_IGS_STAMP(0);
    constexpr int WPN = NWV / 2;
    constexpr int RND = 8 * NWV;
    constexpr int BK = 64;
    constexpr int RWP = BC % RND;
    static_assert(RWP % 8 == 0, "partial round must be whole waves");
    constexpr int RX = BP / RND, RW = (BC + RND - 1) / RND;
    constexpr int L = 2 * (RX + RW);
    constexpr int FP = BP / WPN / 16;
    constexpr int FC = BC / 32;
    constexpr int PLANE = (BP + BC) * 128;
    constexpr int STAGE = 2 * PLANE;
    static_assert(BP % RND == 0 && (BP / WPN) % 16 == 0 && BC % 32 == 0 && 2 * STAGE <= 160 * 1024, "tile");

    extern __shared__ __attribute__((aligned(16))) char smem[];

    const int tid = threadIdx.x;
    const int lane = tid & 63;
    const int wave = __builtin_amdgcn_readfirstlane(tid >> 6);
    const int lr = lane & 15, lg = lane >> 4;
    const int wp = wave % WPN, wc = wave / WPN;
    const int rr = 8 * wave + (lane >> 3);
    const int kcp = (lane & 7) ^ ((lane >> 3) & 7);
    const bool wpart = !RWP || wave < RWP / 8;

    const int nby = (p.Cout + BC - 1) / BC;
    const int tile = xcd_remap(blockIdx.x, gridDim.x);
    const int m0 = (tile / nby) * BP;
    const int n0 = (tile % nby) * BC;
    const long long z = blockIdx.z;
    const bool split = p.splitk > 1;

    constexpr unsigned INV = 0xF0000000u;
    const f16* x0 = (const f16*)p.x0 + (split ? 0 : 2 * z * p.bs_x0);
    const f16* w = (const f16*)p.w + (split ? 0 : 2 * z * p.bs_w);
    const __amdgpu_buffer_rsrc_t rx = __builtin_amdgcn_make_buffer_rsrc((void*)x0, 0, p.x_bytes, 0x00020000);
    const __amdgpu_buffer_rsrc_t rw = __builtin_amdgcn_make_buffer_rsrc((void*)w, 0, p.w_bytes, 0x00020000);

    const int Ctot = p.C0;
    const int ntaps = p.KH * p.KW;
    const int Hv = p.Hs * p.up, Wv = p.Ws * p.up;
    const int ush = p.up == 2 ? 1 : 0;
    const int HoWo = p.Ho * p.Wo;
    const unsigned xlo = (unsigned)p.ld0 * 2u;
    const unsigned wlo = (unsigned)p.Ktot * 2u;

    int pixbase[RX], iy0[RX], ix0[RX];
#pragma unroll
    for (int i = 0; i < RX; ++i) {
        const int m = m0 + RND * i + rr;
        if (m < p.M) {
            int b, rem, oy, ox;
            if (p.sh_wo >= 0) {
                b = m >> p.sh_howo; rem = m & (HoWo - 1); oy = rem >> p.sh_wo; ox = rem & (p.Wo - 1);
            } else {
                b = m / HoWo; rem = m - b * HoWo; oy = rem / p.Wo; ox = rem - oy * p.Wo;
            }
            pixbase[i] = b * p.Hs * p.Ws;
            iy0[i] = oy * p.stride - p.pad_t;
            ix0[i] = ox * p.stride - p.pad_l;
        } else {
            pixbase[i] = -1; iy0[i] = 0; ix0[i] = 0;
// ... 390 lines not shown
        p.sh_wo = pow2 ? __builtin_ctz(p.Wo) : -1;
    }
    float* const want_stats = p.ystats;
    const GNTail want_tail = p.tail;
    if (want_tail.coef && !want_stats) return hipErrorInvalidValue;
    if (want_stats) {
        const int hw = p.Ho * p.Wo;
        if (!std::is_same<TO, h2s>::value || nz != 1) return hipErrorInvalidValue;
        if (p.splitk > 1) { p.ystats = nullptr; p.tail.coef = nullptr; }
        else {
            if ((p.M % BP) || (hw % BP)) return hipErrorInvalidValue;
            if (p.tail.coef) {
                if (p.tail.C > 2048 || p.tail.groups < 1 || p.tail.groups > 64 || (p.tail.C % p.tail.groups)) return hipErrorInvalidValue;
                const int classes = p.osc == 2 ? 4 : 1;
                p.tail.expected = classes * (hw / BP) * ((p.Cout + BC - 1) / BC);
                p.tail.st0 = p.ystats; p.tail.S0 = classes * (hw / BP); p.tail.ld0 = p.ystats_ld; p.tail.n0 = p.Cout;
            }
        }
    }
    hipLaunchKernelGGL((igemm_split_kernel<TO, BP, BC, NWV, PIPE, ABL>), dim3(tiles, 1, p.splitk > 1 ? p.splitk : nz), dim3(64 * NWV), lds, st, p);
    if (p.splitk > 1) {
        p.ystats = want_stats; p.tail = want_tail;
        const int out_dt = std::is_same<TO, h2s>::value ? RS_F16S : RS_F32;
        if ((want_stats ? rs_splitk_reduce_stats_launch(&p, out_dt, st) : rs_splitk_reduce_launch(&p, out_dt, st)) != 0) return hipErrorLaunchFailure;
    }
    return hipGetLastError();
}

template <typename TO, int BP, int BC, int NWV>
hipError_t launch_cfg(const IGemmParams& p, int nz, hipStream_t st) {
#ifdef RS_SPLIT_ABLATE
    if constexpr (std::is_same<TO, h2s>::value && NWV == 8) {
        static const int abl = []() { const char* e = getenv("RS_IGEMM_DBG"); return e ? atoi(e) : 0; }();
        switch (abl) {
            case 1: return launch_cfg2<TO, BP, BC, NWV, true, 1>(p, nz, st);
            case 2: return launch_cfg2<TO, BP, BC, NWV, true, 2>(p, nz, st);
            case 4: return launch_cfg2<TO, BP, BC, NWV, true, 4>(p, nz, st);
            case 6: return launch_cfg2<TO, BP, BC, NWV, true, 6>(p, nz, st);
            default: break;
        }
    }
#endif
    return launch_cfg2<TO, BP, BC, NWV, true>(p, nz, st);
}

template <typename TO>
hipError_t launch_t(const IGemmParams& p, int BP, int BC, int nz, hipStream_t st) {
    if (BP == 64) {
        switch (BC) {
            case 64: return launch_cfg<TO, 64, 64, 4>(p, nz, st);
            case 160: return launch_cfg<TO, 64, 160, 4>(p, nz, st);
            case 192: return launch_cfg<TO, 64, 192, 4>(p, nz, st);
            default: return launch_cfg<TO, 64, 128, 4>(p, nz, st);
        }
    }
    switch (BC) {
        case 64: return launch_cfg<TO, 128, 64, 8>(p, nz, st);
        case 160: return launch_cfg<TO, 128, 160, 8>(p, nz, st);
        case 192: return launch_cfg<TO, 128, 192, 8>(p, nz, st);
        default: return launch_cfg<TO, 128, 128, 8>(p, nz, st);
    }
}

}

extern "C" void rs_igemm_split_pick(int M, int Cout, int nz, int* BP, int* BC) {
    auto waste = [&](int bc) { return ((Cout + bc - 1) / bc) * bc - Cout; };
    int best = 128, bw = waste(128);
    if (waste(160) < bw) { best = 160; bw = waste(160); }
    if (waste(192) < bw) { best = 192; bw = waste(192); }
    if (Cout <= 64) best = 64;
    *BC = best;
    const long long tiles128 = (long long)((M + 127) / 128) * ((Cout + best - 1) / best) * nz;
    *BP = (tiles128 < 256) ? 64 : 128;
    static const int bp128_min = []() { const char* e = getenv("RS_SPLIT_BP128_SK"); return e ? atoi(e) : 64; }();
    if (bp128_min > 0 && nz == 1 && tiles128 >= bp128_min) *BP = 128;
}

extern "C" int rs_igemm_split_stats_px(const IGemmParams* pp, int splitk) {
    const IGemmParams& p = *pp;
    if (p.C1 != 0 || (p.Cout & 3) || (p.ldy & 3)) return 0;
    const int hw = p.Ho * p.Wo;
    if (splitk > 1) return (hw > 256 && (hw % 256)) ? 0 : std::min(hw, 256);
    int BP, BC;
    rs_igemm_split_pick(p.M, p.Cout, 1, &BP, &BC);
    return ((p.M % BP) || (hw % BP)) ? 0 : BP;
}

#ifdef RS_SPLIT_ABLATE
extern "C" int rs_igemm_split_phase_cycles(int nwg, double* out3) {
    static long long h[4 * 8192];
    if (nwg < 1 || nwg > 8192) return -1;
    (void)hipDeviceSynchronize();
    if (hipMemcpyFromSymbol(h, HIP_SYMBOL(g_igs_clk), sizeof(long long) * 4 * nwg) != hipSuccess) return -1;
    out3[0] = out3[1] = out3[2] = 0.0;
    for (int i = 0; i < nwg; ++i)
        for (int k = 0; k < 3; ++k) out3[k] += (double)(h[4 * i + k + 1] - h[4 * i + k]) / nwg;
    return 0;
}
#endif

extern "C" int rs_igemm_split_launch(const IGemmParams* pp, int out_dt, int nz, hipStream_t st) {
    const IGemmParams& p = *pp;
    if (p.C1 != 0 || (p.C0 % 8) || (p.ld0 % 8) || (p.Ktot % 8)) return -2;
    int BP, BC;
    rs_igemm_split_pick(p.M, p.Cout, nz, &BP, &BC);
    hipError_t e;
    if (out_dt == RS_F16S) e = launch_t<h2s>(p, BP, BC, nz, st);
    else if (out_dt == RS_F32) e = launch_t<float>(p, BP, BC, nz, st);
    else return -2;
    return e == hipSuccess ? 0 : -1;
}
```

### resshift_amd/engine.py

```python
from __future__ import annotations

import ctypes as C
from typing import Dict, Mapping, Optional, Sequence

import numpy as np
import torch

from . import _lib
from .spec import _listify, unet_heads

F16, F32, SPLIT = _lib.RS_PREC_F16, _lib.RS_PREC_F32, _lib.RS_PREC_SPLIT
PRECISIONS = {"fp16": F16, "f16": F16, "half": F16, "fp32": F32, "f32": F32, "float": F32, "exact": F32, "split": SPLIT,
              "fp16x3": SPLIT}


def parse_precision(p) -> int:
    if isinstance(p, str):
        return PRECISIONS[p.lower()]
    return int(p)


def _fill_unet(cu: _lib.UNetConfig, p: Mapping) -> None:
    mult = [int(m) for m in p.get("channel_mult", (1, 2, 4, 8))]
    nrb = _listify(p["num_res_blocks"], len(mult))
# ... 321 lines not shown

    def sample(self, y, noise, tables: Dict[str, np.ndarray], sf: int, scale_factor: float, mask=None, prec_unet=F16, prec_encode=F16,
               prec_decode=F16, return_aux=False, keys=None):
        y = self._f32c(y)
        B, _, h, w = y.shape
        steps = int(len(tables["coef1"]))
        f = 2 ** (int(self.cfg.ae.n_levels) - 1)
        hz, wz, cz = h * sf // f, w * sf // f, int(self.cfg.ae.embed_dim)
        karr = self._keys(keys, noise, B, "sample") if keys is not None else None
        if karr is None:
            noise = self._f32c(noise)
            assert tuple(noise.shape) == (steps + 1, B, cz, hz, wz), (tuple(noise.shape), (steps + 1, B, cz, hz, wz))
        out = torch.empty(B, int(self.cfg.ae.out_ch), h * sf, w * sf, device=y.device, dtype=torch.float32)
        a = _lib.SampleArgs()
        mk = self._f32c(mask) if mask is not None else None
        z_out = torch.empty(B, cz, hz, wz, device=y.device, dtype=torch.float32) if return_aux else None
        idx = torch.empty(B * hz * wz, device=y.device, dtype=torch.int32) if return_aux else None
        a.y, a.noise, a.out = y.data_ptr(), (noise.data_ptr() if karr is None else None), out.data_ptr()
        a.mask = mk.data_ptr() if mk is not None else None
        a.z_out = z_out.data_ptr() if z_out is not None else None
        a.idx_out = idx.data_ptr() if idx is not None else None
        a.B, a.h, a.w, a.sf, a.steps = B, h, w, int(sf), steps
        pu = [prec_unet] * steps if isinstance(prec_unet, (int, str)) else list(prec_unet)
        for t in range(steps):
            a.inv_std[t] = float(tables["inv_std"][t])
            a.coef1[t] = float(tables["coef1"][t])
            a.coef2[t] = float(tables["coef2"][t])
            a.sigma[t] = float(tables["sigma"][t])
            a.tmap[t] = int(tables["tmap"][t])
            a.prec_unet[t] = parse_precision(pu[t])
        a.prior_scale = float(tables["prior_scale"])
        a.scale_factor = float(scale_factor)
        a.prec_encode, a.prec_decode = parse_precision(prec_encode), parse_precision(prec_decode)
        a.stream = self._stream()
        with torch.cuda.device(self.device):
            rc = self.lib.rs_sample(self._h, C.byref(a)) if karr is None else self.lib.rs_sample_seeded(self._h, C.byref(a), karr)
        self._chk(rc, "rs_sample" if karr is None else "rs_sample_seeded")
        if return_aux:
            return out, {"z_final": z_out, "indices": idx}
        return out

    def profile_enable(self, on: bool = True):
        self.lib.rs_profile_enable(self._h, int(on))

    def profile_get(self) -> Dict[str, float]:
        out = (C.c_double * 9)()
        self.lib.rs_profile_get(self._h, out)
        return {"flops_f16": out[0], "flops_f32": out[1], "igemm_ms": out[2], "igemm_launches": int(out[3]), "igemm_bytes": out[4],
                "flops_split": out[5], "gn_ms": out[6], "gn_launches": int(out[7]), "gn_bytes": out[8]}

    FAMILIES = ("igemm4_kernel<*, false> (halo 3x3 conv, fp16)", "igemm4_kernel<*, true> (halo 3x3 conv, split storage)",
                "igemm2 / igemm3 / igemm_kernel (implicit GEMM, fp16)", "igemm_split_kernel (implicit GEMM, split storage)",
                "igemm2 / igemm_kernel<float> (implicit GEMM, exact fp32)", "win_attn_qkv_kernel (fused qkv + window attention + proj)",
                "swin_mlp_kernel (fused fc1 + GELU + fc2)", "win_attn_qkv_split_kernel (fused qkv + window attention + proj, split storage)",
                "swin_mlp_split_kernel (fused fc1 + GELU + fc2, split storage)", "ae_flash_attn_kernel (streaming AE mid-block attention, fp16)",
                "ae_flash_attn_split_kernel (streaming AE mid-block attention, split storage)",
                "wino_kernel (Winograd F(2x2,3x3) 3x3 conv, split storage; RS_WINO=1)")

    def profile_families(self):
        out = (C.c_double * (3 * len(self.FAMILIES)))()
        n = self.lib.rs_profile_families(self._h, out, 3 * len(self.FAMILIES))
        return [(self.FAMILIES[f], out[3 * f], out[3 * f + 1], int(out[3 * f + 2])) for f in range(max(0, n))]

    def profile_shapes(self):
        need = self.lib.rs_profile_shapes(self._h, None, 0)
        if need <= 1:
            return [], {}
        buf = C.create_string_buffer(need)
        self.lib.rs_profile_shapes(self._h, buf, need)
        shapes, parts = [], {}
        for line in buf.value.decode().splitlines():
            f = line.split()
            if f and f[0] == "shape" and len(f) >= 10:
                kv = dict(x.split("=") for x in f[3:])
                shapes.append({"part": f[1], "family": int(f[2][1:]), "M": int(kv["M"]), "N": int(kv["N"]), "K": int(kv["K"]), "z": int(kv["z"]),
                               "launches": int(float(kv["n"])), "ms": float(kv["ms"]), "flops": float(kv["flops"])})
            elif f and f[0] == "part":
                parts[f[1]] = float(f[2].split("=")[1])
        return shapes, parts

    def debug_enable(self, on: bool = True):
        self._chk(self.lib.rs_debug_enable(self._h, int(on)), "rs_debug_enable")

    def debug_trace(self, names=None, images=None):
        out = {}
        want = None if names is None else set(names)
        for i in range(self.lib.rs_debug_count(self._h)):
            name = C.create_string_buffer(128)
            dims = (C.c_int * 4)()
            self.lib.rs_debug_info(self._h, i, name, 128, dims)
            key = name.value.decode()
            if want is not None and key not in want:
                continue
            if images is None:
                t = torch.empty(dims[0], dims[1], dims[2], dims[3], device=self.device, dtype=torch.float32)
                self._chk(self.lib.rs_debug_fetch(self._h, i, t.data_ptr(), self._stream()), "rs_debug_fetch")
            else:
                t = torch.empty(len(images), dims[1], dims[2], dims[3], device=self.device, dtype=torch.float32)
                for k, b in enumerate(images):
                    self._chk(self.lib.rs_debug_fetch_rows(self._h, i, int(b), 1, t[k].data_ptr(), self._stream()), "rs_debug_fetch_rows")
            out[key] = t
        torch.cuda.synchronize(self.device)
        return out

    def debug_records(self):
        out = []
        for i in range(self.lib.rs_debug_count(self._h)):
            name = C.create_string_buffer(128)
            dims = (C.c_int * 4)()
            self.lib.rs_debug_info(self._h, i, name, 128, dims)
            out.append((name.value.decode(), tuple(int(d) for d in dims)))
        return out

    def arena_bytes(self) -> int:
        return int(self.lib.rs_arena_bytes(self._h))

    def last_launch_count(self) -> int:
        return int(self.lib.rs_last_launch_count(self._h))
```

### resshift_amd/ops.py

```python
from __future__ import annotations

import ctypes as C

import torch

from . import _lib

F16, F32, SPLIT = _lib.RS_PREC_F16, _lib.RS_PREC_F32, _lib.RS_PREC_SPLIT


def _dt(prec: int) -> torch.dtype:
    return {F16: torch.float16, F32: torch.float32, SPLIT: torch.int32}[prec]


def _prec_of(t: torch.Tensor) -> int:
    return {torch.float16: F16, torch.float32: F32, torch.int32: SPLIT}[t.dtype]


def convert(x, prec):
    lib = _lib.load()
    x = x.contiguous()
    Cc = x.shape[-1]
    out = torch.empty(x.shape, device=x.device, dtype=_dt(prec))
    _lib.check(lib.rs_op_convert(x.data_ptr(), _prec_of(x), out.data_ptr(), prec, Cc, x.numel() // Cc, _lib.current_stream_ptr()), "convert")
    return out


def _hostf(t: torch.Tensor):
    t = t.detach().to("cpu", torch.float32).contiguous()
    return t, t.data_ptr()


def conv2d(x0, w_ref, bias=None, x1=None, res=None, stride=1, pad=(1, 1), out_hw=None, up=1, act=0, out_prec=None,
           force_direct=False):
    lib = _lib.load()
    in_prec = _prec_of(x0)
    out_prec = in_prec if out_prec is None else out_prec
    B, Hs, Ws, C0 = x0.shape
    C1 = 0 if x1 is None else x1.shape[-1]
    Cout, Cin, KH, KW = w_ref.shape
    assert Cin == C0 + C1
    pad_t, pad_l = pad
    if out_hw is None:
        Ho = (Hs * up + 2 * pad_t - KH) // stride + 1
        Wo = (Ws * up + 2 * pad_l - KW) // stride + 1
    else:
        Ho, Wo = out_hw
    y = torch.empty(B, Ho, Wo, Cout, device=x0.device, dtype=_dt(out_prec))
    wh, wp = _hostf(w_ref)
    bh, bp = _hostf(bias) if bias is not None else (None, None)
    rc = lib.rs_op_conv2d(x0.data_ptr(), x1.data_ptr() if x1 is not None else None, wp, bp,
                          res.data_ptr() if res is not None else None, y.data_ptr(), B, Hs, Ws, C0, C1, Cout, KH, KW, stride,
                          pad_t, pad_l, Ho, Wo, up, act, in_prec, out_prec, int(force_direct), _lib.current_stream_ptr())
    _lib.check(rc, "rs_op_conv2d")
    return y


def conv3x3_halo(x, w_ref, bias=None, coef=None, act_in=0, res=None, want_stats=False):
    lib = _lib.load()
    B, H, W, Cin = x.shape
    Cout = w_ref.shape[0]
    prec = _prec_of(x)
    y = torch.empty(B, H, W, Cout, device=x.device, dtype=x.dtype)
    wh, wp = _hostf(w_ref)
    bh, bp = _hostf(bias) if bias is not None else (None, None)
    st = None
    if want_stats:
        spx = lib.rs_op_conv3x3_halo_stats_px(B, H, W, Cin, Cout, prec)
        if spx <= 0:
            raise RuntimeError("this shape gets no output statistics from the halo kernel")
        st = torch.zeros(B, (H * W) // spx, Cout, 2, device=x.device, dtype=torch.float32)
    rc = lib.rs_op_conv3x3_halo(x.data_ptr(), coef.data_ptr() if coef is not None else None, act_in, wp, bp,
                                res.data_ptr() if res is not None else None, y.data_ptr(), B, H, W, Cin, Cout, prec,
                                st.data_ptr() if st is not None else None, _lib.current_stream_ptr())
    _lib.check(rc, "rs_op_conv3x3_halo")
    return (y, st) if want_stats else y


def conv3x3_wino(x, w_ref, bias=None, coef=None, act_in=0, res=None, want_stats=False, reps=0):
    lib = _lib.load()
    B, H, W, Cin = x.shape
    Cout = w_ref.shape[0]
    if _prec_of(x) != 2:
        raise RuntimeError("the wino kernel takes split storage")
    y = torch.empty(B, H, W, Cout, device=x.device, dtype=x.dtype)
    wh, wp = _hostf(w_ref)
    bh, bp = _hostf(bias) if bias is not None else (None, None)
    st = torch.zeros(B, (H * W) // 128, Cout, 2, device=x.device, dtype=torch.float32) if want_stats else None
    ms = C.c_float(0.0)
    rc = lib.rs_op_conv3x3_wino(x.data_ptr(), coef.data_ptr() if coef is not None else None, act_in, wp, bp,
                                res.data_ptr() if res is not None else None, y.data_ptr(), B, H, W, Cin, Cout,
                                st.data_ptr() if st is not None else None, reps, C.byref(ms), _lib.current_stream_ptr())
    _lib.check(rc, "rs_op_conv3x3_wino")
    out = (y, st) if want_stats else y
    return (out, ms.value) if reps > 0 else out


def gemm_nt(a, b, bias=None, scale=1.0, out_prec=None):
    lib = _lib.load()
    in_prec = _prec_of(a)
    out_prec = in_prec if out_prec is None else out_prec
    nz, M, K = a.shape
    N = b.shape[1]
    y = torch.empty(nz, M, N, device=a.device, dtype=_dt(out_prec))
    rc = lib.rs_op_gemm_nt(a.data_ptr(), b.data_ptr(), bias.data_ptr() if bias is not None else None, y.data_ptr(), nz, M, N, K,
                           float(scale), in_prec, out_prec, _lib.current_stream_ptr())
    _lib.check(rc, "rs_op_gemm_nt")
    return y


def groupnorm(x, gamma, beta, eps, act=0, film=None, groups=32):
    lib = _lib.load()
    prec = _prec_of(x)
    B, H, W, Cc = x.shape
    y = torch.empty_like(x)
    gh, gp = _hostf(gamma)
    bh, bp = _hostf(beta)
    rc = lib.rs_op_groupnorm(x.data_ptr(), y.data_ptr(), gp, bp, film.data_ptr() if film is not None else None, B, H * W, Cc, groups,
                             float(eps), act, prec, _lib.current_stream_ptr())
    _lib.check(rc, "rs_op_groupnorm")
    return y


def window_attention(qkv, table, heads, shift):
    lib = _lib.load()
    prec = _prec_of(qkv)
    B, H, W, _ = qkv.shape
    out = torch.empty(B, H, W, heads * 32, device=qkv.device, dtype=qkv.dtype)
    th, tp = _hostf(table)
    rc = lib.rs_op_window_attention(qkv.data_ptr(), out.data_ptr(), tp, B, H, W, heads, shift, prec, _lib.current_stream_ptr())
    _lib.check(rc, "rs_op_window_attention")
    return out


def window_attention_qkv(x, wqkv, bqkv, table, heads, shift, wproj=None, bproj=None, res=None):
    lib = _lib.load()
    B, H, W, E = x.shape
    wd = wqkv.to(x.device, torch.float16).contiguous()
    bd = bqkv.to(x.device, torch.float32).contiguous()
    wpd = wproj.to(x.device, torch.float16).contiguous() if wproj is not None else None
    bpd = bproj.to(x.device, torch.float32).contiguous() if bproj is not None else None
    out = torch.empty(B, H, W, E, device=x.device, dtype=torch.float16)
    th, tp = _hostf(table)
    rc = lib.rs_op_window_attention_qkv(x.data_ptr(), wd.data_ptr(), bd.data_ptr(), wpd.data_ptr() if wpd is not None else None,
                                        bpd.data_ptr() if bpd is not None else None, res.data_ptr() if res is not None else None, out.data_ptr(),
                                        tp, B, H, W, heads, shift, _lib.current_stream_ptr())
    _lib.check(rc, "rs_op_window_attention_qkv")
    return out


def window_attention_qkv_split(x, wqkv, bqkv, table, heads, shift, wproj=None, bproj=None, res=None, xcoef=None):
    lib = _lib.load()
    B, H, W, E = x.shape
    wd = split_pack_rows(wqkv).to(x.device)
    bd = bqkv.to(x.device, torch.float32).contiguous()
    wpd = split_pack_rows(wproj).to(x.device) if wproj is not None else None
    bpd = bproj.to(x.device, torch.float32).contiguous() if bproj is not None else None
    xc = xcoef.to(x.device, torch.float32).contiguous() if xcoef is not None else None
    out = torch.empty(B, H, W, E, device=x.device, dtype=torch.int32)
    th, tp = _hostf(table)
    rc = lib.rs_op_window_attention_qkv_split(x.data_ptr(), wd.data_ptr(), bd.data_ptr(), wpd.data_ptr() if wpd is not None else None,
                                              bpd.data_ptr() if bpd is not None else None, res.data_ptr() if res is not None else None,
                                              out.data_ptr(), tp, xc.data_ptr() if xc is not None else None, B, H, W, heads, shift,
                                              _lib.current_stream_ptr())
    _lib.check(rc, "rs_op_window_attention_qkv_split")
    return out


def ae_flash_attention(q, k, v, bv=None):
    lib = _lib.load()
    nz, T, C = q.shape
    vt = v.transpose(1, 2).contiguous()
    bd = bv.to(q.device, torch.float32).contiguous() if bv is not None else None
    o = torch.empty_like(q)
    rc = lib.rs_op_ae_flash_attention(q.contiguous().data_ptr(), k.contiguous().data_ptr(), vt.data_ptr(), bd.data_ptr() if bd is not None else None,
                                      o.data_ptr(), nz, T, C, _lib.current_stream_ptr())
    _lib.check(rc, "rs_op_ae_flash_attention")
    return o


# ... 109 lines not shown
```

Measured before the change: 134.8 images/sec.

## Add persistent weight-resident streaming conv kernel for split-precision 1x1 and stem convs

Adds a persistent kernel for split-precision (hi/lo fp16) convolutions. Each workgroup keeps one Cout panel of the weights in LDS and streams many 128-pixel tiles through a register ring buffer, with the GroupNorm statistics/tail fused in. It covers 1x1 convs with K of 64-320 and the 3x3 conv with 8 input channels, on large spatial maps without residual or activation, and the igemm dispatcher now routes those shapes here instead of the split igemm. The aim is to stop reloading weights per tile and cut launch and tile overhead on memory-bound convs. The cost is a new dispatch path, fewer workgroups (one per CU per panel), and changed stats granularity (stats_px becomes 128), which downstream GN consumers must respect.

Result: no change. 135.3 images/sec (median of 6 runs) (+0.4%).

```diff
diff --git a/include/resshift_hip.h b/include/resshift_hip.h
--- a/include/resshift_hip.h
+++ b/include/resshift_hip.h
@@ -152,6 +152,7 @@
 int rs_profile_families(rs_engine* e, double* out, int cap);
 int rs_profile_shapes(rs_engine* e, char* buf, int cap);
 int rs_debug_enable(rs_engine* e, int on);
+int rs_debug_no_stream(rs_engine* e, int on);
 int rs_debug_count(rs_engine* e);
 int rs_debug_info(rs_engine* e, int i, char* name, int name_cap, int* dims_bchw);
 int rs_debug_fetch(rs_engine* e, int i, float* out_nchw_dev, void* stream);
@@ -168,6 +169,12 @@
 int rs_op_conv3x3_wino(const void* x, const float* coef_dev, int act_in, const float* w_ref_host, const float* bias_host, const void* res,
                        void* y, int B, int H, int W, int Cin, int Cout, float* ystats_dev, int reps, float* ms_out, void* stream);
 int rs_op_conv3x3_halo_stats_px(int B, int H, int W, int Cin, int Cout, int prec);
+int rs_op_conv_stream(const void* x, const float* w_ref_host, const float* bias_host, const void* res, void* y, int B, int H, int W, int Cin,
+                      int Cout, int KH, int stride, int act, int out_prec, float* ystats_dev, const float* tail_gamma_host,
+                      const float* tail_beta_host, float tail_eps, int tail_groups, float* tail_coef_dev, int force_generic, int max_wgs, int reps,
+                      float* ms_out, void* stream);
+int rs_op_conv_stream_plan(int B, int H, int W, int Cin, int Cout, int KH, int stride, int has_res, int act, int out_prec, int force_generic,
+                           int op_level, int* stats_px);
 int rs_op_gemm_nt(const void* a, const void* b, const float* bias_dev, void* y, int nz, int M, int N, int K, float scale,
                   int in_prec, int out_prec, void* stream);
 int rs_op_groupnorm(const void* x, void* y, const float* gamma_host, const float* beta_host, const float* film_dev, int B, int HW,
diff --git a/resshift_amd/_lib.py b/resshift_amd/_lib.py
--- a/resshift_amd/_lib.py
+++ b/resshift_amd/_lib.py
@@ -137,6 +137,7 @@
     "rs_profile_families": (_I, [_P, C.POINTER(C.c_double), _I]),
     "rs_profile_shapes": (_I, [_P, C.c_char_p, _I]),
     "rs_debug_enable": (_I, [_P, _I]),
+    "rs_debug_no_stream": (_I, [_P, _I]),
     "rs_debug_count": (_I, [_P]),
     "rs_debug_info": (_I, [_P, _I, C.c_char_p, _I, C.POINTER(C.c_int)]),
     "rs_debug_fetch": (_I, [_P, _I, _P, _P]),
@@ -146,6 +147,8 @@
     "rs_op_conv3x3_halo_stats_px": (_I, [_I, _I, _I, _I, _I, _I]),
     "rs_op_conv3x3_halo": (_I, [_P, _P, _I, _P, _P, _P, _P, _I, _I, _I, _I, _I, _I, _P, _P]),
     "rs_op_conv3x3_wino": (_I, [_P, _P, _I, _P, _P, _P, _P, _I, _I, _I, _I, _I, _P, _I, C.POINTER(C.c_float), _P]),
+    "rs_op_conv_stream": (_I, [_P, _P, _P, _P, _P] + [_I] * 9 + [_P, _P, _P, _F, _I, _P, _I, _I, _I, C.POINTER(C.c_float), _P]),
+    "rs_op_conv_stream_plan": (_I, [_I] * 12 + [C.POINTER(C.c_int)]),
     "rs_op_gemm_nt": (_I, [_P, _P, _P, _P, _I, _I, _I, _I, _F, _I, _I, _P]),
     "rs_op_groupnorm": (_I, [_P, _P, _P, _P, _P, _I, _I, _I, _I, _F, _I, _I, _P]),
     "rs_op_window_attention": (_I, [_P, _P, _P, _I, _I, _I, _I, _I, _I, _P]),
diff --git a/resshift_amd/build.py b/resshift_amd/build.py
--- a/resshift_amd/build.py
+++ b/resshift_amd/build.py
@@ -10,7 +10,7 @@
 CSRC = os.path.join(HERE, "csrc")
 OBJ = os.path.join(CSRC, "build" + ("_" + hashlib.sha256(os.environ["RS_BUILD_DEFS"].encode()).hexdigest()[:8] if os.environ.get("RS_BUILD_DEFS") else ""))
 LIB = os.environ.get("RS_BUILD_OUT") or os.path.join(HERE, "libresshift_hip.so")
-SOURCES = ["igemm.hip", "igemm2.hip", "igemm3.hip", "igemm4.hip", "igemm4s.hip", "wino.hip", "igemm_split.hip", "swin_mlp.hip", "direct_conv.hip", "norm_attn.hip", "win_attn_split.hip", "ae_attn.hip", "ae_attn_split.hip", "elementwise.hip", "colorfix.hip", "engine.hip"]
+SOURCES = ["igemm.hip", "igemm2.hip", "igemm3.hip", "igemm4.hip", "igemm4s.hip", "wino.hip", "igemm_split.hip", "stream_conv.hip", "swin_mlp.hip", "direct_conv.hip", "norm_attn.hip", "win_attn_split.hip", "ae_attn.hip", "ae_attn_split.hip", "elementwise.hip", "colorfix.hip", "engine.hip"]
 HEADERS = ["common.h", "igemm_common.h", "igemm4_kernel.h", "gn_tail.h", "philox.h", os.path.join("..", "..", "include", "resshift_hip.h")]
 HIPCC = os.environ.get("HIPCC", "/opt/rocm/bin/hipcc")
 FLAGS = ["--offload-arch=gfx950", "-O3", "-std=c++17", "-fPIC", "-Wno-unused-result"]
diff --git a/resshift_amd/csrc/common.h b/resshift_amd/csrc/common.h
--- a/resshift_amd/csrc/common.h
+++ b/resshift_amd/csrc/common.h
@@ -188,6 +188,7 @@
     unsigned sx_bytes, sw_bytes;
     int osc, ooy, oox;
     const void* ww;
+    int no_stream, stream_wgs;
 };
 
 #if defined(__HIPCC__)
diff --git a/resshift_amd/csrc/engine.hip b/resshift_amd/csrc/engine.hip
--- a/resshift_amd/csrc/engine.hip
+++ b/resshift_amd/csrc/engine.hip
@@ -25,6 +25,7 @@
 int rs_wino_stats_px();
 int rs_wino_tiles(const IGemmParams* p);
 int rs_igemm_split_stats_px(const IGemmParams* p, int splitk);
+int rs_stream_conv_plan(const IGemmParams* p, int out_dt, int nz);
 int rs_direct_conv_launch(const DirectConvParams* p, int in_dt, int out_dt, hipStream_t st);
 int rs_head_conv_launch(const void* x, int in_dt, const float* coef_dev, const float* w_dev, const float* bias_dev, float* y, int B, int H, int W, int C,
                         int ldx, int Cout, int ldy, hipStream_t st);
@@ -406,6 +407,7 @@
     std::string last_shapes;
     long long last_igemm_launches = 0, last_gn_launches = 0;
     bool debug = false;
+    bool no_stream = false;
     std::vector<TraceRec> trace;
     rs_noise_key* keys_dev = nullptr; size_t keys_cap = 0;
     const rs_noise_key* stage_keys(const rs_noise_key* keys, int B, hipStream_t st) {
@@ -917,8 +919,8 @@
         return (blob.off + 255) & ~(size_t)255;
     }
 
-    static IGemmParams conv_params(const ConvW& w, const View& x, const View* x1, const View& y, int stride, int pad_t, int pad_l, int up,
-                                   int act, const View* res, float out_scale) {
+    IGemmParams conv_params(const ConvW& w, const View& x, const View* x1, const View& y, int stride, int pad_t, int pad_l, int up,
+                            int act, const View* res, float out_scale) const {
         const int C1 = x1 ? x1->C : 0;
         IGemmParams p{};
         p.x0 = x.p; p.x1 = x1 ? x1->p : nullptr; p.w = w.w_for(x.dt); p.bias = w.bias;
@@ -929,6 +931,7 @@
         p.M = y.B * y.H * y.W; p.Ktot = w.KH * w.KW * (x.C + C1); p.act = act; p.out_scale = out_scale;
         p.splitk = 1;
         p.ww = (x.dt == RS_F16S && !x1) ? w.ww : nullptr;
+        p.no_stream = no_stream ? 1 : 0;
         return p;
     }
     bool halo_conv(const ConvW& w, const View& x, const View& y, const View* res, int* sk = nullptr, int* seg = nullptr, bool folded = false,
@@ -2003,6 +2006,11 @@
         e->free_capture();
     }
     e->trace.clear();
+    return 0;
+}
+int rs_debug_no_stream(rs_engine* e, int on) {
+    if (!e) return -1;
+    e->no_stream = on != 0;
     return 0;
 }
 int rs_debug_count(rs_engine* e) { return e ? (int)e->trace.size() : 0; }
@@ -2476,6 +2484,90 @@
     return rc;
 }
 
+static IGemmParams conv_stream_params(int B, int H, int W, int Cin, int Cout, int KH, int stride) {
+    const int pad = KH == 3 ? 1 : 0;
+    IGemmParams p{};
+    p.C0 = Cin; p.ld0 = Cin; p.B = B; p.Hs = H; p.Ws = W; p.up = 1; p.Ho = (H + 2 * pad - KH) / stride + 1; p.Wo = (W + 2 * pad - KH) / stride + 1;
+    p.KH = KH; p.KW = KH; p.stride = stride; p.pad_t = pad; p.pad_l = pad; p.Cout = Cout; p.ldy = Cout; p.ldres = Cout; p.M = B * p.Ho * p.Wo;
+    p.Ktot = KH * KH * Cin; p.out_scale = 1.f; p.splitk = 1;
+    return p;
+}
+int rs_op_conv_stream_plan(int B, int H, int W, int Cin, int Cout, int KH, int stride, int has_res, int act, int out_prec, int force_generic, int op_level,
+                           int* stats_px) {
+    IGemmParams p = conv_stream_params(B, H, W, Cin, Cout, KH, stride);
+    p.res = has_res ? (const void*)&p : nullptr;
+    p.act = act; p.no_stream = force_generic; p.dbg = op_level ? 64 : 0;
+    p.splitk = rs_igemm_splitk_plan(p.M, Cout, p.Ktot, RS_F16S);
+    int tw, bc;
+    const bool other = rs_wino_plan(&p, RS_F16S, out_prec, 1) || rs_igemm4_pick(&p, RS_F16S, out_prec, 1, &tw, &bc);
+    if (stats_px) *stats_px = (out_prec == RS_F16S && !other) ? rs_igemm_split_stats_px(&p, p.splitk) : 0;
+    return !other && rs_stream_conv_plan(&p, out_prec, 1);
+}
+int rs_op_conv_stream(const void* x, const float* w_ref_host, const float* bias_host, const void* res, void* y, int B, int H, int W, int Cin, int Cout,
+                      int KH, int stride, int act, int out_prec, float* ystats_dev, const float* tail_gamma_host, const float* tail_beta_host,
+                      float tail_eps, int tail_groups, float* tail_coef_dev, int force_generic, int max_wgs, int reps, float* ms_out, void* stream) {
+    hipStream_t st = (hipStream_t)stream;
+    if ((KH != 1 && KH != 3) || (Cin % 8)) return fail("conv_stream: 1x1 or 3x3, input channels in multiples of 8");
+    const int T = KH * KH;
+    const size_t K = (size_t)T * Cin, n = K * Cout;
+    std::vector<f16> o(2 * n);
+    for (int co = 0; co < Cout; ++co)
+        for (int ci = 0; ci < Cin; ++ci)
+            for (int t = 0; t < T; ++t) {
+                f16 h, l;
+                rs_split(w_ref_host[((size_t)co * Cin + ci) * T + t], h, l);
+                o[(size_t)co * 2 * K + (size_t)t * Cin + ci] = h;
+                o[(size_t)co * 2 * K + K + (size_t)t * Cin + ci] = l;
+            }
+    void* wdev = dev_copy(o.data(), o.size() * 2);
+    float* bias = bias_host ? (float*)dev_copy(bias_host, Cout * 4) : nullptr;
+    IGemmParams p = conv_stream_params(B, H, W, Cin, Cout, KH, stride);
+    p.x0 = x; p.w = wdev; p.bias = bias; p.res = res; p.y = y; p.act = act;
+    p.no_stream = force_generic ? 1 : 0; p.stream_wgs = max_wgs; p.dbg = 64;
+    p.splitk = rs_igemm_splitk_plan(p.M, Cout, (int)K, RS_F16S);
+    float* part = nullptr;
+    if (p.splitk > 1) { (void)hipMalloc((void**)&part, (size_t)p.splitk * p.M * Cout * sizeof(float)); p.partial = part; }
+    p.ystats = ystats_dev; p.ystats_ld = Cout;
+    float *g = nullptr, *bt = nullptr;
+    unsigned* ticket = nullptr;
+    int rc = 0;
+    if (tail_coef_dev) {
+        if (!ystats_dev || !tail_gamma_host || !tail_beta_host) rc = fail("conv_stream: a tail needs statistics, gamma and beta");
+        else {
+            g = (float*)dev_copy(tail_gamma_host, Cout * 4); bt = (float*)dev_copy(tail_beta_host, Cout * 4);
+            (void)hipMalloc((void**)&ticket, (size_t)B * sizeof(unsigned));
+            (void)hipMemsetAsync(ticket, 0, (size_t)B * sizeof(unsigned), st);
+            p.tail.gamma = g; p.tail.beta = bt; p.tail.eps = tail_eps; p.tail.groups = tail_groups; p.tail.C = Cout; p.tail.HW = p.Ho * p.Wo;
+            p.tail.coef = tail_coef_dev; p.tail.ticket = ticket;
+        }
+    }
+    if (!rc) {
+        rc = rs_igemm_launch(&p, RS_F16S, out_prec, 1, st);
+        if (rc) fail("igemm launch rejected the shape");
+    }
+    if (!rc && reps > 0) {
+        p.tail = GNTail{};
+        hipEvent_t e0, e1;
+        (void)hipEventCreate(&e0); (void)hipEventCreate(&e1);
+        (void)hipEventRecord(e0, st);
+        for (int i = 0; i < reps; ++i) rc |= rs_igemm_launch(&p, RS_F16S, out_prec, 1, st);
+        (void)hipEventRecord(e1, st);
+        (void)hipEventSynchronize(e1);
+        float ms = 0.f;
+        (void)hipEventElapsedTime(&ms, e0, e1);
+        if (ms_out) *ms_out = ms / (float)reps;
+        (void)hipEventDestroy(e0); (void)hipEventDestroy(e1);
+    }
+    (void)hipStreamSynchronize(st);
+    if (part) (void)hipFree(part);
+    if (ticket) (void)hipFree(ticket);
+    if (g) (void)hipFree(g);
+    if (bt) (void)hipFree(bt);
+    if (wdev) (void)hipFree(wdev);
+    if (bias) (void)hipFree(bias);
+    return rc;
+}
+
 int rs_op_conv3x3_halo_stats_px(int B, int H, int W, int Cin, int Cout, int prec) {
     IGemmParams p{};
     p.C0 = Cin; p.ld0 = Cin; p.B = B; p.Hs = H; p.Ws = W; p.up = 1; p.Ho = H; p.Wo = W;
diff --git a/resshift_amd/csrc/igemm.hip b/resshift_amd/csrc/igemm.hip
--- a/resshift_amd/csrc/igemm.hip
+++ b/resshift_amd/csrc/igemm.hip
@@ -340,6 +340,8 @@
 extern "C" int rs_wino_launch(const IGemmParams* pp, hipStream_t st);
 extern "C" void rs_igemm_split_pick(int M, int Cout, int nz, int* BP, int* BC);
 extern "C" int rs_igemm_split_launch(const IGemmParams* pp, int out_dt, int nz, hipStream_t st);
+extern "C" int rs_stream_conv_plan(const IGemmParams* pp, int out_dt, int nz);
+extern "C" int rs_stream_conv_launch(const IGemmParams* pp, hipStream_t st);
 
 extern "C" int rs_splitk_reduce_launch(const IGemmParams* pp, int out_dt, hipStream_t st) {
     const IGemmParams& p = *pp;
@@ -393,6 +395,7 @@
         if (rs_igemm4_pick(&p, in_dt, out_dt, nz, &tw4, &bc4)) return rs_igemm4_launch(&p, in_dt, tw4, bc4, st);
         if (p.xcoef || p.sx) return -2;
     }
+    if (in_dt == RS_F16S && rs_stream_conv_plan(&p, out_dt, nz)) return rs_stream_conv_launch(&p, st);
     if (in_dt == RS_F16S) return rs_igemm_split_launch(&p, out_dt, nz, st);
     static const bool use_v2 = []() { const char* e = getenv("RS_IGEMM_V2"); return !(e && e[0] == '0'); }();
     int bp2 = 0, bc2 = 0;
diff --git a/resshift_amd/csrc/igemm_split.hip b/resshift_amd/csrc/igemm_split.hip
--- a/resshift_amd/csrc/igemm_split.hip
+++ b/resshift_amd/csrc/igemm_split.hip
@@ -5,6 +5,7 @@
 
 extern "C" int rs_splitk_reduce_launch(const IGemmParams* p, int out_dt, hipStream_t st);
 extern "C" int rs_splitk_reduce_stats_launch(const IGemmParams* p, int out_dt, hipStream_t st);
+extern "C" int rs_stream_conv_plan(const IGemmParams* pp, int out_dt, int nz);
 
 namespace {
 
@@ -561,6 +562,7 @@
     if (p.C1 != 0 || (p.Cout & 3) || (p.ldy & 3)) return 0;
     const int hw = p.Ho * p.Wo;
     if (splitk > 1) return (hw > 256 && (hw % 256)) ? 0 : std::min(hw, 256);
+    if (rs_stream_conv_plan(pp, RS_F16S, 1)) return 128;
     int BP, BC;
     rs_igemm_split_pick(p.M, p.Cout, 1, &BP, &BC);
     return ((p.M % BP) || (hw % BP)) ? 0 : BP;
diff --git a/resshift_amd/csrc/stream_conv.hip b/resshift_amd/csrc/stream_conv.hip
--- /dev/null
+++ b/resshift_amd/csrc/stream_conv.hip
@@ -0,0 +1,326 @@
+#include "igemm_common.h"
+#include "gn_tail.h"
+#include <algorithm>
+
+extern "C" int rs_stream_conv_plan(const IGemmParams* pp, int out_dt, int nz);
+
+namespace {
+
+using namespace igemm_detail;
+
+constexpr int SC_NWV = 8;
+constexpr int SC_BP = 128;
+constexpr int SC_LIST = 64;
+constexpr int SC_TAIL_C = 1280;
+constexpr unsigned SC_INV = 0xF0000000u;
+
+struct StreamPlan {
+    int NP;
+    int npanel;
+    int P0;
+    int pitch;
+    int G;
+    int ntiles;
+    int nks, maxp;
+    size_t lds;
+};
+
+__device__ __forceinline__ f16x8 ld16(__amdgpu_buffer_rsrc_t r, unsigned off) {
+    return __builtin_bit_cast(f16x8, __builtin_amdgcn_raw_buffer_load_b128(r, (int)off, 0, 0));
+}
+
+template <int NKS, int D, int MAXP, bool CONV3>
+__global__ __launch_bounds__(64 * SC_NWV, 2) void stream_conv_kernel(IGemmParams p, StreamPlan s) {
+    constexpr int WCH = MAXP * 32;
+    extern __shared__ __attribute__((aligned(16))) char smem[];
+
+    const int tid = threadIdx.x;
+    const int lane = tid & 63;
+    const int wave = __builtin_amdgcn_readfirstlane(tid >> 6);
+    const int lr = lane & 15, lg = lane >> 4;
+    const int wp = wave & 3, wc = wave >> 2;
+
+    const int v = xcd_remap(blockIdx.x, gridDim.x);
+    const int panel = v % s.npanel, g = v / s.npanel;
+    const int n0 = panel * s.NP;
+    const int t_begin = (int)((long long)g * s.ntiles / s.G), t_end = (int)((long long)(g + 1) * s.ntiles / s.G);
+    const int npair = wc ? s.NP / 32 - s.P0 : s.P0;
+    const int cbase = wc ? s.P0 * 32 : 0;
+
+    char* const wlo_s = smem + s.NP * s.pitch;
+    float* const sb = (float*)(smem + 2 * s.NP * s.pitch);
+    int* const lst = (int*)(sb + 2 * SC_NWV * WCH * 2);
+    float* const tscr = (float*)(lst + 1 + SC_LIST);
+
+    const __amdgpu_buffer_rsrc_t rx = __builtin_amdgcn_make_buffer_rsrc((void*)p.x0, 0, p.x_bytes, 0x00020000);
+    const int K = p.Ktot, kch = K >> 3;
+    const int HoWo = p.Ho * p.Wo;
+    const unsigned xlo = (unsigned)p.ld0 * 2u;
+    const unsigned rec = (unsigned)p.ld0 * 4u;
+
+    static_assert(NKS % D == 0, "ring");
+    f16x8 bh[D][2], bl[D][2];
+    struct Loc {
+        unsigned base[2];
+        int pb[2], py[2], px[2];
+    };
+    Loc cur, nxt;
+    auto locate = [&](int tile, Loc& L) {
+#pragma unroll
+        for (int j = 0; j < 2; ++j) {
+            const int m = tile * SC_BP + wp * 32 + j * 16 + lr;
+            if constexpr (CONV3) {
+                const int b = m / HoWo, rem = m - b * HoWo;
+                L.py[j] = rem / p.Wo; L.px[j] = rem - L.py[j] * p.Wo; L.pb[j] = b * HoWo;
+            } else {
+                L.base[j] = (unsigned)m * rec + (unsigned)lg * 16u;
+            }
+        }
+    };
+    auto issue = [&](int ks, const Loc& L) __attribute__((always_inline)) {
+        const int c = ks * 4 + lg;
+#pragma unroll
+        for (int j = 0; j < 2; ++j) {
+            unsigned off;
+            if constexpr (CONV3) {
+                const int ky = c / 3, kx = c - ky * 3;
+                const int iy = L.py[j] + ky - 1, ix = L.px[j] + kx - 1;
+                const bool ok = c < 9 && (unsigned)iy < (unsigned)p.Hs && (unsigned)ix < (unsigned)p.Ws;
+                off = ok ? (unsigned)(L.pb[j] + iy * p.Ws + ix) * rec : SC_INV;
+            } else {
+                off = c < kch ? L.base[j] + (unsigned)ks * 64u : SC_INV;
+            }
+            bh[ks % D][j] = ld16(rx, off);
+            bl[ks % D][j] = ld16(rx, off == SC_INV ? SC_INV : off + xlo);
+        }
+    };
+
+    locate(t_begin, nxt);
+    if (t_begin < t_end) {
+#pragma unroll
+        for (int ks = 0; ks < D; ++ks) issue(ks, nxt);
+    }
+    {
+        const f16* w = (const f16*)p.w;
+        const int per = 2 * kch;
+        for (int idx = tid; idx < s.NP * per; idx += 64 * SC_NWV) {
+            const int row = idx / per, c = idx - row * per;
+            const int half = c >= kch ? 1 : 0, cc = c - half * kch;
+            const int ch = (row & ~31) + ((row & 15) >> 2) * 8 + ((row >> 4) & 1) * 4 + (row & 3);
+            const uint4 q = *(const uint4*)(w + ((long long)(n0 + ch) * 2 * K + (long long)c * 8));
+            *(uint4*)(smem + half * (s.NP * s.pitch) + row * s.pitch + cc * 16) = q;
+        }
+        if (tid == 0) lst[0] = 0;
+    }
+    const int arow = cbase + lr;
+    const char* const a_hi = smem + arow * s.pitch + lg * 16;
+    const char* const a_lo = wlo_s + arow * s.pitch + lg * 16;
+    f32x4 bvs[MAXP][2];
+#pragma unroll
+    for (int t = 0; t < MAXP; ++t)
+#pragma unroll
+        for (int e = 0; e < 2; ++e) {
+            bvs[t][e] = f32x4{0.f, 0.f, 0.f, 0.f};
+            if (p.bias && t < npair) bvs[t][e] = *(const f32x4*)(p.bias + n0 + cbase + t * 32 + lg * 8 + e * 4);
+        }
+    __syncthreads();
+
+    f16* const y = (f16*)p.y;
+    int nlast = 0;
+    for (int tile = t_begin; tile < t_end; ++tile) {
+        const bool more = tile + 1 < t_end;
+        cur = nxt;
+        if (more) locate(tile + 1, nxt);
+        f32x4 am[2 * MAXP][2], ac[2 * MAXP][2];
+#pragma unroll
+        for (int i = 0; i < 2 * MAXP; ++i)
+#pragma unroll
+            for (int j = 0; j < 2; ++j) { am[i][j] = f32x4{0.f, 0.f, 0.f, 0.f}; ac[i][j] = f32x4{0.f, 0.f, 0.f, 0.f}; }
+#pragma unroll
+        for (int ks = 0; ks < NKS; ++ks) {
+            const bool aval = ks * 4 + lg < kch;
+            const bool apart = ks * 4 + 4 > kch;
+#pragma unroll
+            for (int t = 0; t < MAXP; ++t) {
+                if (t < npair) {
+                    f16x8 ah[2], al[2];
+#pragma unroll
+                    for (int e = 0; e < 2; ++e) {
+                        const int o = (t * 32 + e * 16) * s.pitch + ks * 64;
+                        ah[e] = *(const f16x8*)(a_hi + o);
+                        al[e] = *(const f16x8*)(a_lo + o);
+                        if (apart && !aval) { ah[e] = f16x8{0, 0, 0, 0, 0, 0, 0, 0}; al[e] = f16x8{0, 0, 0, 0, 0, 0, 0, 0}; }
+                    }
+#pragma unroll
+                    for (int e = 0; e < 2; ++e) {
+#pragma unroll
+                        for (int j = 0; j < 2; ++j) am[2 * t + e][j] = __builtin_amdgcn_mfma_f32_16x16x32_f16(ah[e], bh[ks % D][j], am[2 * t + e][j], 0, 0, 0);
+#pragma unroll
+                        for (int j = 0; j < 2; ++j) ac[2 * t + e][j] = __builtin_amdgcn_mfma_f32_16x16x32_f16(ah[e], bl[ks % D][j], ac[2 * t + e][j], 0, 0, 0);
+#pragma unroll
+                        for (int j = 0; j < 2; ++j) ac[2 * t + e][j] = __builtin_amdgcn_mfma_f32_16x16x32_f16(al[e], bh[ks % D][j], ac[2 * t + e][j], 0, 0, 0);
+                    }
+                }
+            }
+            if (ks + D < NKS) issue(ks + D, cur);
+            else if (more) issue(ks + D - NKS, nxt);
+        }
+
+#pragma unroll
+        for (int i = 0; i < 2 * MAXP; ++i)
+#pragma unroll
+            for (int j = 0; j < 2; ++j) {
+#pragma unroll
+                for (int r = 0; r < 4; ++r) am[i][j][r] = fmaf(ac[i][j][r], RS_LO_INV, am[i][j][r]);
+                const f32x4 q = am[i][j] * p.out_scale + bvs[i >> 1][i & 1];
+                am[i][j] = q;
+            }
+        const int m0 = tile * SC_BP;
+        if (p.ystats) {
+            float* const sbt = sb + (tile & 1) * (SC_NWV * WCH * 2);
+#pragma unroll
+            for (int t = 0; t < MAXP; ++t) {
+                if (t < npair) {
+#pragma unroll
+                    for (int e = 0; e < 2; ++e)
+#pragma unroll
+                        for (int r = 0; r < 4; ++r) {
+                            float a = 0.f, q = 0.f;
+#pragma unroll
+                            for (int j = 0; j < 2; ++j) { a += am[2 * t + e][j][r]; q = fmaf(am[2 * t + e][j][r], am[2 * t + e][j][r], q); }
+                            a = rs_sum16(a); q = rs_sum16(q);
+                            const int cl = t * 32 + lg * 8 + e * 4 + r;
+                            if (lr == 0) { sbt[(wave * WCH + cl) * 2] = a; sbt[(wave * WCH + cl) * 2 + 1] = q; }
+                        }
+                }
+            }
+            __syncthreads();
+            if (wave == 0) {
+                const int img = m0 / HoWo;
+                for (int c = lane; c < s.NP; c += 64) {
+                    const int hw_ = c >= s.P0 * 32 ? 1 : 0, cl = c - hw_ * s.P0 * 32;
+                    float a = 0.f, q = 0.f;
+#pragma unroll
+                    for (int w4 = 0; w4 < 4; ++w4) { a += sbt[((hw_ * 4 + w4) * WCH + cl) * 2]; q += sbt[((hw_ * 4 + w4) * WCH + cl) * 2 + 1]; }
+                    float* dst = p.ystats + ((long long)(m0 / SC_BP) * p.ystats_ld + n0 + c) * 2;
+                    if (p.tail.coef) rs_pub_pair(dst, a, q);
+                    else { dst[0] = a; dst[1] = q; }
+                }
+                if (p.tail.coef) {
+                    const bool last = rs_gn_tail_arrive(p.tail, img);
+                    if (last) { if (lane == 0 && nlast < SC_LIST) lst[1 + nlast] = img; ++nlast; }
+                }
+            }
+        }
+#pragma unroll
+        for (int t = 0; t < MAXP; ++t) {
+            if (t < npair) {
+#pragma unroll
+                for (int j = 0; j < 2; ++j) {
+                    f16x8 h, l;
+#pragma unroll
+                    for (int e = 0; e < 2; ++e)
+#pragma unroll
+                        for (int r = 0; r < 4; ++r) { f16 a, b; rs_split(am[2 * t + e][j][r], a, b); h[e * 4 + r] = a; l[e * 4 + r] = b; }
+                    const long long m = m0 + wp * 32 + j * 16 + lr;
+                    f16* yp = y + m * p.ldy * 2 + n0 + cbase + t * 32 + lg * 8;
+                    *(f16x8*)yp = h;
+                    *(f16x8*)(yp + p.ldy) = l;
+                }
+            }
+        }
+    }
+    if (p.ystats && p.tail.coef) {
+        if (wave == 0 && lane == 0) lst[0] = min(nlast, SC_LIST);
+        __syncthreads();
+        const int n = lst[0];
+        for (int i = 0; i < n; ++i) {
+            rs_gn_tail_finish<64 * SC_NWV>(p.tail, lst[1 + i], tscr);
+            __syncthreads();
+        }
+    }
+}
+
+int cu_count() {
+    static int n[RS_MAX_DEVICES + 1] = {};
+    const int s = rs_device_slot();
+    if (n[s] > 0) return n[s];
+    int v = 0, d = 0;
+    if (hipGetDevice(&d) != hipSuccess || hipDeviceGetAttribute(&v, hipDeviceAttributeMultiprocessorCount, d) != hipSuccess || v <= 0) v = 256;
+    if (s < RS_MAX_DEVICES) n[s] = v;
+    return v;
+}
+
+bool plan_shape(const IGemmParams& p, int out_dt, int nz, StreamPlan& s) {
+    if (out_dt != RS_F16S || nz != 1 || p.no_stream || p.splitk > 1 || p.osc != 0 || p.up != 1 || p.C1 != 0 || p.x1 || p.res || p.act != RS_ACT_NONE) return false;
+    if (p.xcoef || p.sx || p.stride != 1 || p.Ho != p.Hs || p.Wo != p.Ws || p.B * p.Ho * p.Wo != p.M) return false;
+    if (p.Ho * p.Wo < 1024 && !(p.dbg & 64)) return false;
+    if (p.M <= 0 || (p.M % SC_BP) || ((p.Ho * p.Wo) % SC_BP) || (p.Cout % 32) || (p.ldy % 8) || (p.ld0 % 8)) return false;
+    const int K = p.Ktot;
+    bool conv3 = false;
+    if (p.KH == 1 && p.KW == 1 && p.pad_t == 0 && p.pad_l == 0) {
+        if (K != p.C0 || K < 64 || K > 320 || (K % 8)) return false;
+    } else if (p.KH == 3 && p.KW == 3 && p.pad_t == 1 && p.pad_l == 1) {
+        if (p.C0 != 8 || K != 72) return false;
+        conv3 = true;
+    } else return false;
+    const int nk = (K + 63) / 64;
+    if (nk != 2 && nk != 3 && nk != 5) return false;
+    if (conv3 && nk != 2) return false;
+    if ((size_t)p.B * p.Hs * p.Ws * p.ld0 * 4 >= 0xF0000000ull) return false;
+    if (p.tail.coef && (!p.ystats || p.tail.C > SC_TAIL_C || p.tail.groups < 1 || p.tail.groups > 64 || (p.tail.C % p.tail.groups))) return false;
+    s.nks = 2 * nk;
+    s.pitch = (K / 8 + 1 + ((K / 8) & 1)) * 16;
+    static const int cand[] = {192, 160, 128, 96, 64, 32};
+    for (int np : cand) {
+        if (p.Cout % np) continue;
+        const int pairs = np / 32, P0 = (pairs + 1) / 2, maxp = P0 <= 2 ? 2 : 3;
+        const size_t lds = (size_t)2 * np * s.pitch + (size_t)2 * SC_NWV * maxp * 32 * 2 * sizeof(float) + (1 + SC_LIST) * sizeof(int)
+                           + (size_t)(2 * SC_TAIL_C + 2 * 64) * sizeof(float);
+        if (lds > 160 * 1024) continue;
+        s.NP = np; s.npanel = p.Cout / np; s.P0 = P0; s.maxp = maxp; s.lds = lds; s.ntiles = p.M / SC_BP;
+        return true;
+    }
+    return false;
+}
+
+template <int NKS, int D, int MAXP, bool CONV3>
+hipError_t launch_k(const IGemmParams& p, const StreamPlan& s, hipStream_t st) {
+    static RsAttrFlags attr_flags;
+    if (attr_flags.need()) (void)hipFuncSetAttribute((const void*)stream_conv_kernel<NKS, D, MAXP, CONV3>, hipFuncAttributeMaxDynamicSharedMemorySize, 160 * 1024);
+    hipLaunchKernelGGL((stream_conv_kernel<NKS, D, MAXP, CONV3>), dim3(s.G * s.npanel), dim3(64 * SC_NWV), s.lds, st, p, s);
+    return hipGetLastError();
+}
+
+}
+
+extern "C" int rs_stream_conv_plan(const IGemmParams* pp, int out_dt, int nz) {
+    StreamPlan s{};
+    return plan_shape(*pp, out_dt, nz, s) ? 1 : 0;
+}
+
+extern "C" int rs_stream_conv_launch(const IGemmParams* pp, hipStream_t st) {
+    IGemmParams p = *pp;
+    StreamPlan s{};
+    if (!plan_shape(p, RS_F16S, 1, s)) return -2;
+    p.x_bytes = (unsigned)((size_t)p.B * p.Hs * p.Ws * p.ld0 * 4);
+    int G = std::max(1, cu_count() / s.npanel);
+    if (p.stream_wgs > 0) G = std::max(1, p.stream_wgs / s.npanel);
+    G = std::min(G, s.ntiles);
+    G = std::max(G, (s.ntiles + SC_LIST - 1) / SC_LIST);
+    s.G = G;
+    if (p.ystats && p.tail.coef) {
+        const int hw = p.Ho * p.Wo;
+        p.tail.expected = (hw / SC_BP) * s.npanel;
+        p.tail.st0 = p.ystats; p.tail.S0 = hw / SC_BP; p.tail.ld0 = p.ystats_ld; p.tail.n0 = p.Cout;
+    } else {
+        p.tail.coef = nullptr;
+    }
+    const bool conv3 = p.KH == 3;
+    hipError_t e;
+    if (conv3) e = s.maxp == 2 ? launch_k<4, 4, 2, true>(p, s, st) : launch_k<4, 4, 3, true>(p, s, st);
+    else if (s.nks == 4) e = s.maxp == 2 ? launch_k<4, 4, 2, false>(p, s, st) : launch_k<4, 4, 3, false>(p, s, st);
+    else if (s.nks == 6) e = s.maxp == 2 ? launch_k<6, 6, 2, false>(p, s, st) : launch_k<6, 6, 3, false>(p, s, st);
+    else e = s.maxp == 2 ? launch_k<10, 5, 2, false>(p, s, st) : launch_k<10, 5, 3, false>(p, s, st);
+    return e == hipSuccess ? 0 : -1;
+}
diff --git a/resshift_amd/engine.py b/resshift_amd/engine.py
--- a/resshift_amd/engine.py
+++ b/resshift_amd/engine.py
@@ -427,6 +427,9 @@
     def debug_enable(self, on: bool = True):
         self._chk(self.lib.rs_debug_enable(self._h, int(on)), "rs_debug_enable")
 
+    def debug_no_stream(self, on: bool = True):
+        self._chk(self.lib.rs_debug_no_stream(self._h, int(on)), "rs_debug_no_stream")
+
     def debug_trace(self, names=None, images=None):
         out = {}
         want = None if names is None else set(names)
diff --git a/resshift_amd/ops.py b/resshift_amd/ops.py
--- a/resshift_amd/ops.py
+++ b/resshift_amd/ops.py
@@ -96,6 +96,54 @@
     return (out, ms.value) if reps > 0 else out
 
 
+def conv_stream_plan(B, H, W, Cin, Cout, ksize=1, stride=1, has_res=False, act=0, out_prec=SPLIT, force_generic=False, op_level=False):
+    lib = _lib.load()
+    spx = C.c_int(0)
+    acc = lib.rs_op_conv_stream_plan(B, H, W, Cin, Cout, ksize, stride, int(has_res), act, out_prec, int(force_generic), int(op_level), C.byref(spx))
+    return int(acc), int(spx.value)
+
+
+def conv_stream(x, w_ref, bias=None, want_stats=False, coef_tail=None, force_generic=False, max_wgs=0, res=None, stride=1, act=0,
+                out_prec=SPLIT, reps=0):
+    lib = _lib.load()
+    if _prec_of(x) != SPLIT:
+        raise RuntimeError("conv_stream takes split storage")
+    B, H, W, Cin = x.shape
+    Cout, _, k, _ = w_ref.shape
+    pad = 1 if k == 3 else 0
+    Ho, Wo = (H + 2 * pad - k) // stride + 1, (W + 2 * pad - k) // stride + 1
+    y = torch.empty(B, Ho, Wo, Cout, device=x.device, dtype=_dt(out_prec))
+    wh, wp = _hostf(w_ref)
+    bh, bp = _hostf(bias) if bias is not None else (None, None)
+    st = coef = None
+    gp = btp = None
+    eps, groups = 0.0, 0
+    if want_stats or coef_tail is not None:
+        _, spx = conv_stream_plan(B, H, W, Cin, Cout, k, stride, res is not None, act, out_prec, force_generic, True)
+        if spx <= 0:
+            raise RuntimeError("this launch leaves no output statistics")
+        st = torch.zeros(B, (Ho * Wo) // spx, Cout, 2, device=x.device, dtype=torch.float32)
+    if coef_tail is not None:
+        gamma, beta, eps, groups = coef_tail
+        gh, gp = _hostf(gamma)
+        bth, btp = _hostf(beta)
+        coef = torch.zeros(B, 2, Cout, device=x.device, dtype=torch.float32)
+    ms = C.c_float(0.0)
+    rc = lib.rs_op_conv_stream(x.data_ptr(), wp, bp, res.data_ptr() if res is not None else None, y.data_ptr(), B, H, W, Cin, Cout, k, stride,
+                               act, out_prec, st.data_ptr() if st is not None else None, gp, btp, float(eps), int(groups),
+                               coef.data_ptr() if coef is not None else None, int(force_generic), int(max_wgs), int(reps), C.byref(ms),
+                               _lib.current_stream_ptr())
+    _lib.check(rc, "rs_op_conv_stream")
+    out = [y]
+    if want_stats:
+        out.append(st)
+    if coef_tail is not None:
+        out.append(coef)
+    if reps > 0:
+        out.append(ms.value)
+    return out[0] if len(out) == 1 else tuple(out)
+
+
 def gemm_nt(a, b, bias=None, scale=1.0, out_prec=None):
     lib = _lib.load()
     in_prec = _prec_of(a)
```
